# Arlo0o/StereoScene

Hardware: AMD Instinct MI355X
Metric: voxels/sec fwd+bwd, 256x256x32 grid D=192 (higher is better)
Workload: dtype f32; 1 GPU; kitti_d192: stereo pair features 2x[B,640,48,160] -> 256x256x32 occupancy, D=192, fwd+bwd incl. 4 losses; batch_per_gpu=1, global_batch=1, parallelism=dp1, train_mode=True

## Files before the change

include/ssbev.h:

```cpp
#ifndef SSBEV_H
#define SSBEV_H

#include <stddef.h>
#include <stdint.h>

#ifdef __cplusplus
extern "C" {
#endif

#define SSBEV_OK 0
#define SSBEV_EINVAL (-1)
#define SSBEV_EWORKSPACE (-2)
#define SSBEV_ELAUNCH (-3)

typedef void* ssbev_stream_t;

int ssbev_version(void);
const char* ssbev_build_arch(void);
void ssbev_env_refresh(void);

typedef struct {
  int B;
  int P;
  int C;
// ... 39 lines not shown
typedef struct { int B, C, G, D, H, W; float down; int align_corners; } ssbev_gwc_dims;
int ssbev_gwc_warp_fwd(const float* left, const float* right, const float* calib, float* vol,
                       const ssbev_gwc_dims* d, ssbev_stream_t stream);
int ssbev_gwc_warp_bwd(const float* grad_vol, const float* left, const float* right,
                       const float* calib, float* grad_left, float* grad_right,
                       const ssbev_gwc_dims* d, ssbev_stream_t stream);
size_t ssbev_gwc_warp_bwd_workspace(const ssbev_gwc_dims* d);
int ssbev_gwc_warp_bwd_fused(const float* grad_vol, const float* left, const float* right,
                             const float* calib, float* grad_left, float* grad_right,
                             const ssbev_gwc_dims* d, void* workspace, size_t ws_bytes, ssbev_stream_t stream);

typedef struct {
  int B, Cin, Cout;
  int Di, Hi, Wi;
  int Do, Ho, Wo;
  int kd, kh, kw;
  int sd, sh, sw;
  int pd, ph, pw;
  int dd, dh, dw;
  int transposed;
  int relu;
  int accumulate;
  int tile_hint;
  int precision;
} ssbev_conv_dims;

size_t ssbev_conv_packed_weight_elems(const ssbev_conv_dims* d);
int ssbev_conv_kernel_class(const ssbev_conv_dims* d, int mode);

size_t ssbev_conv_thin_workspace(const ssbev_conv_dims* d, int mode);
size_t ssbev_conv_thin_packed_elems(const ssbev_conv_dims* d, int mode);
int ssbev_conv_thin_pack(const float* w_src, float* w_packed, const ssbev_conv_dims* d, int mode, ssbev_stream_t stream);
int ssbev_conv_thin_run(const float* x, const float* w_packed, const float* bias, float* y, const ssbev_conv_dims* d,
                        int mode, void* workspace, size_t ws_bytes, ssbev_stream_t stream);
int ssbev_conv_pack_weight(const float* w_src, float* w_packed, const ssbev_conv_dims* d, int mode,
                           ssbev_stream_t stream);
int ssbev_conv_fwd(const float* x, const float* w_packed, const float* bias, float* y,
                   const ssbev_conv_dims* d, ssbev_stream_t stream);
int ssbev_conv_fwd_bf16(const uint16_t* x, const float* w_packed, const float* bias, void* y,
                        const ssbev_conv_dims* d, ssbev_stream_t stream);
int ssbev_conv_bwd_data_bf16(const uint16_t* gy, const float* w_packed_t, void* gx,
                             const ssbev_conv_dims* d, ssbev_stream_t stream);
int ssbev_conv_bwd_weight_bf16(const uint16_t* x, const uint16_t* gy, float* gw, const ssbev_conv_dims* d,
                               void* ws, size_t ws_bytes, ssbev_stream_t stream);
int ssbev_conv_bwd_data(const float* gy, const float* w_packed_t, float* gx,
                        const ssbev_conv_dims* d, ssbev_stream_t stream);
size_t ssbev_conv_bwd_weight_workspace(const ssbev_conv_dims* d);
int ssbev_conv_bwd_weight(const float* x, const float* gy, float* gw, const ssbev_conv_dims* d,
                          void* ws, size_t ws_bytes, ssbev_stream_t stream);

typedef struct { int M, N, K, batch; int out_fp32; } ssbev_gemm16_dims;
size_t ssbev_gemm16_packed_elems(const ssbev_gemm16_dims* d);
int ssbev_gemm16_pack(const float* B, uint16_t* packed, const ssbev_gemm16_dims* d, ssbev_stream_t stream);
int ssbev_gemm16_nn(const uint16_t* A, const uint16_t* packed, void* C, const ssbev_gemm16_dims* d, ssbev_stream_t stream);
size_t ssbev_gemm16_tn_workspace(const ssbev_gemm16_dims* d);
int ssbev_gemm16_tn(const uint16_t* A, const uint16_t* B, float* C, const ssbev_gemm16_dims* d, float* workspace,
                    size_t workspace_elems, ssbev_stream_t stream);

typedef struct { int B, C, G; int64_t S; float eps; int relu; int stats_given; int pre_act; int64_t ld_y, ld_gy; int io_dtype; } ssbev_norm_dims;
size_t ssbev_groupnorm_workspace(const ssbev_norm_dims* d);
int ssbev_groupnorm_fwd(const float* x, const float* gamma, const float* beta, const float* residual,
                        float* y, float* mean, float* rstd, const ssbev_norm_dims* d, void* ws,
                        size_t ws_bytes, ssbev_stream_t stream);
int ssbev_groupnorm_bwd(const float* gy, const float* x, const float* y, const float* gamma,
                        const float* mean, const float* rstd, float* gx, float* gresidual,
                        float* ggamma, float* gbeta, const ssbev_norm_dims* d, void* ws,
                        size_t ws_bytes, ssbev_stream_t stream);
size_t ssbev_groupnorm_mask_words(const ssbev_norm_dims* d);
int ssbev_groupnorm_fwd_mask(const float* x, const float* gamma, const float* beta, const float* residual, float* y,
                             float* mean, float* rstd, uint64_t* relu_mask, const ssbev_norm_dims* d, void* ws,
                             size_t ws_bytes, ssbev_stream_t stream);
int ssbev_groupnorm_bwd_mask(const float* gy, const float* x, const uint64_t* relu_mask, const float* gamma,
                             const float* mean, const float* rstd, float* gx, float* gresidual, float* ggamma, float* gbeta,
                             const ssbev_norm_dims* d, void* ws, size_t ws_bytes, ssbev_stream_t stream);

typedef struct { float* running_mean; float* running_var; float momentum; int64_t n; } ssbev_norm_ext;
int ssbev_groupnorm_fwd_ext(const float* x, const float* gamma, const float* beta, const float* residual, float* y,
                            float* mean, float* rstd, uint64_t* relu_mask, const ssbev_norm_dims* d,
                            const ssbev_norm_ext* ext, void* ws, size_t ws_bytes, ssbev_stream_t stream);
int ssbev_groupnorm_bwd_ext(const float* gy, const float* x, const float* y, const uint64_t* relu_mask, const float* gamma,
                            const float* mean, const float* rstd, float* gx, float* gresidual, float* ggamma, float* gbeta,
                            const ssbev_norm_dims* d, const ssbev_norm_ext* ext, void* ws, size_t ws_bytes,
                            ssbev_stream_t stream);

typedef struct { int B, C, Ga, Gb; int64_t S; float eps_a, eps_b; int relu; int a_batch, b_batch; int io_dtype;  } ssbev_norm2_dims;
size_t ssbev_groupnorm2_workspace(const ssbev_norm2_dims* d);
int ssbev_groupnorm2_fwd(const float* xa, const float* gamma_a, const float* beta_a, float* mean_a, float* rstd_a,
                         const float* xb, const float* gamma_b, const float* beta_b, float* mean_b, float* rstd_b, float* y,
                         uint64_t* relu_mask, const ssbev_norm2_dims* d, void* ws, size_t ws_bytes, ssbev_stream_t stream);
int ssbev_groupnorm2_bwd(const float* gy, const uint64_t* relu_mask, const float* xa, const float* gamma_a, const float* mean_a,
                         const float* rstd_a, const float* xb, const float* gamma_b, const float* mean_b, const float* rstd_b,
                         float* gxa, float* gxb, float* ggamma_a, float* gbeta_a, float* ggamma_b, float* gbeta_b,
                         const ssbev_norm2_dims* d, void* ws, size_t ws_bytes, ssbev_stream_t stream);

typedef struct { float* running_mean_a; float* running_var_a; float momentum_a;
                 float* running_mean_b; float* running_var_b; float momentum_b; } ssbev_norm2_ext;
int ssbev_groupnorm2_fwd_ext(const float* xa, const float* gamma_a, const float* beta_a, float* mean_a, float* rstd_a,
                             const float* xb, const float* gamma_b, const float* beta_b, float* mean_b, float* rstd_b, float* y,
                             uint64_t* relu_mask, const ssbev_norm2_dims* d, const ssbev_norm2_ext* ext, void* ws, size_t ws_bytes,
                             ssbev_stream_t stream);
int ssbev_groupnorm2_bwd_ext(const float* gy, const uint64_t* relu_mask, const float* xa, const float* gamma_a, const float* mean_a,
                             const float* rstd_a, const float* xb, const float* gamma_b, const float* mean_b, const float* rstd_b,
                             float* gxa, float* gxb, float* ggamma_a, float* gbeta_a, float* ggamma_b, float* gbeta_b,
                             const ssbev_norm2_dims* d, const ssbev_norm2_ext* ext, void* ws, size_t ws_bytes,
                             ssbev_stream_t stream);

typedef struct { int B, D, H, W, C; } ssbev_upsample_dims;
int ssbev_trilinear2x_fwd(const float* x, float* y, const ssbev_upsample_dims* d, ssbev_stream_t stream);
int ssbev_trilinear2x_bwd(const float* gy, float* gx, const ssbev_upsample_dims* d, ssbev_stream_t stream);

typedef struct { float lr, beta1, beta2, eps, weight_decay, max_grad_norm; int step; } ssbev_adamw_cfg;
size_t ssbev_grad_norm_workspace(void);
int ssbev_grad_norm(const float* g, int64_t n, float* norm_out, void* ws, size_t ws_bytes,
                    ssbev_stream_t stream);
int ssbev_adamw_step(float* p, const float* g, float* m, float* v, int64_t n,
                     const ssbev_adamw_cfg* c, const float* grad_norm, ssbev_stream_t stream);

typedef struct { int B, D, H, W, C; } ssbev_occloss_dims;
int ssbev_occ_loss_num_sums(void);
size_t ssbev_occ_loss_workspace(const ssbev_occloss_dims* d);
int ssbev_occ_loss_fwd(const float* logits, const uint8_t* label, const float* class_weight, double* sums,
                       const ssbev_occloss_dims* d, void* ws, size_t ws_bytes, ssbev_stream_t stream);
int ssbev_bri_shell_chunks(void);
int ssbev_bri_shell_pre_fwd(const float* q, const float* kv, const float* conf, const float* wq, const float* bq,
                            const float* wk, const float* bk, const float* wv, const float* bv, float* Q, float* K, float* Vc,
                            int B, int D, int T, ssbev_stream_t stream);
int ssbev_bri_shell_post_fwd(const float* out, const float* kv, const float* gamma, float* y, int B, int D, int T,
                             ssbev_stream_t stream);
int ssbev_bri_shell_post_bwd(const float* gy, const float* out, const float* gamma, float* gout, float* delta_part, double* part,
                             int B, int D, int T, ssbev_stream_t stream);
int ssbev_bri_shell_pre_bwd(const float* gQ, const float* gK, const float* gVc, const float* q, const float* kv, const float* conf,
                            const float* gres, const float* wq, const float* wk, const float* wv, const float* bv, float* gq,
                            float* gkv, float* gconf_part, double* part, int B, int D, int T, ssbev_stream_t stream);

int ssbev_occ_loss_tail(const double* sums, float w_ce, float w_sem, float w_geo, float* out5, double* jac,
                        ssbev_stream_t stream);
size_t ssbev_occ_loss_bwd_workspace(const ssbev_occloss_dims* d);
int ssbev_occ_loss_bwd(const float* logits, const uint8_t* label, const float* class_weight,
                       const float* coef, float* grad_logits, const ssbev_occloss_dims* d, void* ws,
                       size_t ws_bytes, ssbev_stream_t stream);

int ssbev_bn_update_running(const float* mean, const float* rstd, float* running_mean, float* running_var, int C,
                            float momentum, float eps, int64_t n, ssbev_stream_t stream);

int ssbev_softmax_axis_fwd(const float* x, float* y, int64_t outer, int C, int64_t inner, ssbev_stream_t stream);
int ssbev_softmax_axis_bwd(const float* y, const float* gy, float* gx, int64_t outer, int C, int64_t inner,
                           ssbev_stream_t stream);
int ssbev_softmax_rows_fwd(const float* x, float* y, int64_t rows, int C, ssbev_stream_t stream);
int ssbev_softmax_rows_bwd(const float* y, const float* gy, float* gx, int64_t rows, int C, ssbev_stream_t stream);

typedef struct { int B, C, H, W, G, k, pad, dil; } ssbev_dcn_dims;
int ssbev_dcn_im2col(const float* x, const float* offset, float* cols, const ssbev_dcn_dims* d, ssbev_stream_t stream);
size_t ssbev_dcn_col2im_workspace(const ssbev_dcn_dims* d);
int ssbev_dcn_col2im(const float* x, const float* offset, const float* gcols, float* gx, float* goffset,
                     const ssbev_dcn_dims* d, void* ws, size_t ws_bytes, ssbev_stream_t stream);

int ssbev_resize_pil_u8(const uint8_t* src, int Hs, int Ws, int C, const int32_t* kk_h, const int32_t* bounds_h, int ksize_h,
                        const int32_t* kk_v, const int32_t* bounds_v, int ksize_v, uint8_t* tmp, uint8_t* dst, int Hd, int Wd,
                        ssbev_stream_t stream);
int ssbev_crop_normalize_u8(const uint8_t* src, int Hs, int Ws, float* dst, int x0, int y0, int w, int h, int flip,
                            const float* mean, const float* stdinv, int swap_rb, ssbev_stream_t stream);
int ssbev_crop_rotate_normalize_u8(const uint8_t* src, int Hs, int Ws, float* dst, int x0, int y0, int w, int h, int flip,
                                   const int32_t* affine6, const float* mean, const float* stdinv, int swap_rb,
                                   ssbev_stream_t stream);
size_t ssbev_depth_bce_workspace(int BN, int fH, int fW);
int ssbev_depth_bce_fwd(const float* gt_depths, const float* depth_pred, float* out2, int BN, int D, int fH, int fW, int ds,
                        float c0, float dd, float weight, void* ws, size_t ws_bytes, ssbev_stream_t stream);
int ssbev_depth_bce_bwd(const float* depth_pred, const float* grad_loss, const float* out2, float* grad_pred, int BN, int D, int fH,
                        int fW, int ds, float c0, float dd, float weight, const void* ws, ssbev_stream_t stream);

size_t ssbev_lidar_depth_workspace(int H, int W);
int ssbev_lidar_depth_map(const float* points, int n_points, const float* cam, const float* labels, float* uvd,
                          unsigned char* valid, float* depth, float* seg, int H, int W, void* ws, size_t ws_bytes,
                          ssbev_stream_t stream);

typedef struct { int B, C, Hi, Wi, Ho, Wo, k, stride, pad_t, pad_l; } ssbev_dw_dims;
int ssbev_dwconv2d_fwd(const float* x, const float* w, float* y, const ssbev_dw_dims* d, ssbev_stream_t stream);
int ssbev_dwconv2d_bwd_data(const float* gy, const float* w, float* gx, const ssbev_dw_dims* d, ssbev_stream_t stream);
size_t ssbev_dwconv2d_bwd_weight_workspace(const ssbev_dw_dims* d);
int ssbev_dwconv2d_bwd_weight(const float* x, const float* gy, float* gw, const ssbev_dw_dims* d, float* ws,
                              size_t ws_elems, ssbev_stream_t stream);
int ssbev_swish_fwd(const float* x, float* y, int64_t n, ssbev_stream_t stream);
int ssbev_swish_bwd(const float* x, const float* gy, float* gx, int64_t n, ssbev_stream_t stream);
size_t ssbev_chan_sum_workspace(int B, int64_t S, int C);
int ssbev_chan_sum(const float* a, const float* bmul, float* out, int B, int64_t S, int C, float scale, float* ws,
                   size_t ws_elems, ssbev_stream_t stream);
int ssbev_chan_scale(const float* x, const float* gate, float* y, int B, int64_t S, int C, float scale,
                     ssbev_stream_t stream);

typedef struct { int B, D, H, W, C; } ssbev_wino_dims;
int ssbev_wino_input_transform(const float* x, float* V, const ssbev_wino_dims* d, ssbev_stream_t stream);
int ssbev_wino_output_transform(const float* M, float* y, const ssbev_wino_dims* d, ssbev_stream_t stream);
int ssbev_wino_output_adjoint(const float* gy, float* Z, const ssbev_wino_dims* d, ssbev_stream_t stream);
int ssbev_wino2d_input_transform(const float* x, float* V, const ssbev_wino_dims* d, ssbev_stream_t stream);
int ssbev_wino2d_output_transform(const float* M, float* y, const ssbev_wino_dims* d, ssbev_stream_t stream);
int ssbev_wino2d_output_adjoint(const float* gy, float* Z, const ssbev_wino_dims* d, ssbev_stream_t stream);
int ssbev_wino_input_transform_bf16(const float* x, uint16_t* V, const ssbev_wino_dims* d, ssbev_stream_t stream);
int ssbev_wino_output_transform_bf16(const uint16_t* M, float* y, const ssbev_wino_dims* d, ssbev_stream_t stream);
int ssbev_wino_output_adjoint_bf16(const float* gy, uint16_t* Z, const ssbev_wino_dims* d, ssbev_stream_t stream);
int ssbev_wino2d_input_transform_bf16(const float* x, uint16_t* V, const ssbev_wino_dims* d, ssbev_stream_t stream);
int ssbev_wino2d_output_transform_bf16(const uint16_t* M, float* y, const ssbev_wino_dims* d, ssbev_stream_t stream);
int ssbev_wino2d_output_adjoint_bf16(const float* gy, uint16_t* Z, const ssbev_wino_dims* d, ssbev_stream_t stream);
int ssbev_wino_input_transform_bf16a(const uint16_t* x, uint16_t* V, const ssbev_wino_dims* d, ssbev_stream_t stream);
int ssbev_wino_output_transform_bf16a(const uint16_t* M, uint16_t* y, const ssbev_wino_dims* d, ssbev_stream_t stream);
int ssbev_wino_output_adjoint_bf16a(const uint16_t* gy, uint16_t* Z, const ssbev_wino_dims* d, ssbev_stream_t stream);
int ssbev_wino2d_input_transform_bf16a(const uint16_t* x, uint16_t* V, const ssbev_wino_dims* d, ssbev_stream_t stream);
int ssbev_wino2d_output_transform_bf16a(const uint16_t* M, uint16_t* y, const ssbev_wino_dims* d, ssbev_stream_t stream);
int ssbev_wino2d_output_adjoint_bf16a(const uint16_t* gy, uint16_t* Z, const ssbev_wino_dims* d, ssbev_stream_t stream);
int ssbev_wino43_input_transform(const float* x, float* V, const ssbev_wino_dims* d, ssbev_stream_t stream);
int ssbev_wino43_output_transform(const float* M, float* y, const ssbev_wino_dims* d, ssbev_stream_t stream);
int ssbev_wino43_output_adjoint(const float* gy, float* Z, const ssbev_wino_dims* d, ssbev_stream_t stream);
int ssbev_wino43_2d_input_transform(const float* x, float* V, const ssbev_wino_dims* d, ssbev_stream_t stream);
int ssbev_wino43_2d_output_transform(const float* M, float* y, const ssbev_wino_dims* d, ssbev_stream_t stream);
int ssbev_wino43_2d_output_transform_acc(const float* M, float* y, const ssbev_wino_dims* d, ssbev_stream_t stream);
int ssbev_wino2d_output_transform_acc(const float* M, float* y, const ssbev_wino_dims* d, ssbev_stream_t stream);
int ssbev_wino43_2d_output_adjoint(const float* gy, float* Z, const ssbev_wino_dims* d, ssbev_stream_t stream);
int ssbev_wino43_input_transform_bf16(const float* x, uint16_t* V, const ssbev_wino_dims* d, ssbev_stream_t stream);
int ssbev_wino43_output_transform_bf16(const uint16_t* M, float* y, const ssbev_wino_dims* d, ssbev_stream_t stream);
int ssbev_wino43_output_adjoint_bf16(const float* gy, uint16_t* Z, const ssbev_wino_dims* d, ssbev_stream_t stream);
int ssbev_wino43_2d_input_transform_bf16(const float* x, uint16_t* V, const ssbev_wino_dims* d, ssbev_stream_t stream);
int ssbev_wino43_2d_output_transform_bf16(const uint16_t* M, float* y, const ssbev_wino_dims* d, ssbev_stream_t stream);
int ssbev_wino43_2d_output_adjoint_bf16(const float* gy, uint16_t* Z, const ssbev_wino_dims* d, ssbev_stream_t stream);
int ssbev_wino444_input_transform(const float* x, float* V, const ssbev_wino_dims* d, ssbev_stream_t stream);
int ssbev_wino444_output_transform(const float* M, float* y, const ssbev_wino_dims* d, ssbev_stream_t stream);
int ssbev_wino444_output_adjoint(const float* gy, float* Z, const ssbev_wino_dims* d, ssbev_stream_t stream);
int ssbev_wino43_weight_transform(const float* w, float* U, int Cout, int Cin, int ndim, int mode, ssbev_stream_t stream);
int ssbev_wino43_weight_grad(const float* gU, float* gw, int Cout, int Cin, int ndim, ssbev_stream_t stream);
int ssbev_wino_weight_transform(const float* w, float* U, int Cout, int Cin, int ndim, int mode, ssbev_stream_t stream);
int ssbev_wino_weight_grad(const float* gU, float* gw, int Cout, int Cin, int ndim, ssbev_stream_t stream);
size_t ssbev_wino_dgemm_packed_elems(int Cout, int Cin);
int ssbev_wino_dgemm_pack(const float* w, float* Wp, int Cout, int Cin, int mode, ssbev_stream_t stream);
int ssbev_wino_dgemm(const float* P, const float* Wp, float* Mo, const ssbev_wino_dims* d, int N, ssbev_stream_t stream);
int ssbev_wino_bgemm(const float* A, const float* Wp, float* Cm, int64_t T, int K, int N, ssbev_stream_t stream);

typedef struct {
  int M, N, K, batch;
  int64_t lda, ldb, ldc, sa, sb, sc;
  int relu;
  int d2s_D, d2s_H, d2s_W, d2s_kd, d2s_kh, d2s_kw, d2s_Co;
  const int64_t* d2s_rowoff;
  const float* ep_mul;
  const float* ep_rowsub;
} ssbev_gemm_dims;
int ssbev_gemm_d2s_rowoff(int64_t* rowoff, int M, int D, int H, int W, int kd, int kh, int kw, int Co, ssbev_stream_t stream);
size_t ssbev_gemm_nn_workspace(const ssbev_gemm_dims* d);
size_t ssbev_gemm_nt_workspace(const ssbev_gemm_dims* d);
int ssbev_gemm_nn(const float* A, const float* B, const float* bias, float* C, const ssbev_gemm_dims* d, void* workspace,
                  size_t ws_bytes, ssbev_stream_t stream);
int ssbev_gemm_nt(const float* A, const float* W, const float* bias, float* C, const ssbev_gemm_dims* d, void* workspace,
                  size_t ws_bytes, ssbev_stream_t stream);
size_t ssbev_gemm_tn_workspace(const ssbev_gemm_dims* d);
int ssbev_gemm_tn(const float* A, const float* B, float* C, const ssbev_gemm_dims* d, void* workspace, size_t ws_bytes,
                  ssbev_stream_t stream);

int ssbev_wino43_df_supported(const ssbev_wino_dims* d, int N);
int ssbev_wino43_df_instance(const ssbev_wino_dims* d, int N);
size_t ssbev_wino43_df_packed_elems(int Cout, int Cin);
int ssbev_wino43_df_pack(const float* w, float* Wp, int Cout, int Cin, int mode, ssbev_stream_t stream);
int ssbev_wino43_df_gemm(const float* P, const float* Wp, float* Mo, const ssbev_wino_dims* d, int N, ssbev_stream_t stream);
size_t ssbev_wino43_df_wgrad_workspace(const ssbev_wino_dims* d, int N);
int ssbev_wino43_df_wgrad(const float* P, const float* Z, float* gw, const ssbev_wino_dims* d, int N, void* workspace,
                          size_t ws_bytes, ssbev_stream_t stream);

#ifdef __cplusplus
}
#endif
#endif
```

stereoscene_amd/capi.py:

```python
import ctypes as C
import os

import torch

_HERE = os.path.dirname(os.path.abspath(__file__))
LIB_PATH = os.path.join(_HERE, "_lib", "libssbev_hip.so")

OK, EINVAL, EWORKSPACE, ELAUNCH = 0, -1, -2, -3
_ERR = {EINVAL: "SSBEV_EINVAL (bad dims / null pointer / unsupported configuration)",
        EWORKSPACE: "SSBEV_EWORKSPACE (workspace too small)",
        ELAUNCH: "SSBEV_ELAUNCH (HIP launch failure)"}


class SsbevError(RuntimeError):
    pass


class PoolDims(C.Structure):
    _fields_ = [("B", C.c_int), ("P", C.c_int), ("C", C.c_int), ("nx", C.c_int), ("ny", C.c_int), ("nz", C.c_int),
                ("origin", C.c_float * 3), ("dx", C.c_float * 3)]


class LiftDims(C.Structure):
    _fields_ = [("N", C.c_int), ("D", C.c_int), ("HW", C.c_int)]
# ... 37 lines not shown
class Norm2Ext(C.Structure):
    _fields_ = [("running_mean_a", C.c_void_p), ("running_var_a", C.c_void_p), ("momentum_a", C.c_float),
                ("running_mean_b", C.c_void_p), ("running_var_b", C.c_void_p), ("momentum_b", C.c_float)]


class DcnDims(C.Structure):
    _fields_ = [(n, C.c_int) for n in ("B", "C", "H", "W", "G", "k", "pad", "dil")]


class DwDims(C.Structure):
    _fields_ = [(n, C.c_int) for n in ("B", "C", "Hi", "Wi", "Ho", "Wo", "k", "stride", "pad_t", "pad_l")]


class WinoDims(C.Structure):
    _fields_ = [(n, C.c_int) for n in ("B", "D", "H", "W", "C")]


class UpsampleDims(C.Structure):
    _fields_ = [("B", C.c_int), ("D", C.c_int), ("H", C.c_int), ("W", C.c_int), ("C", C.c_int)]


class GemmDims(C.Structure):
    _fields_ = [("M", C.c_int), ("N", C.c_int), ("K", C.c_int), ("batch", C.c_int),
                ("lda", C.c_int64), ("ldb", C.c_int64), ("ldc", C.c_int64), ("sa", C.c_int64), ("sb", C.c_int64), ("sc", C.c_int64),
                ("relu", C.c_int),
                ("d2s_D", C.c_int), ("d2s_H", C.c_int), ("d2s_W", C.c_int), ("d2s_kd", C.c_int), ("d2s_kh", C.c_int),
                ("d2s_kw", C.c_int), ("d2s_Co", C.c_int), ("d2s_rowoff", C.c_void_p),
                ("ep_mul", C.c_void_p), ("ep_rowsub", C.c_void_p)]


class AdamWCfg(C.Structure):
    _fields_ = [("lr", C.c_float), ("beta1", C.c_float), ("beta2", C.c_float), ("eps", C.c_float),
                ("weight_decay", C.c_float), ("max_grad_norm", C.c_float), ("step", C.c_int)]


_P = C.c_void_p
SIGNATURES = {
    "ssbev_version": (C.c_int, []),
    "ssbev_build_arch": (C.c_char_p, []),
    "ssbev_env_refresh": (None, []),
    "ssbev_voxel_index": (C.c_int, [_P, _P, _P, C.POINTER(PoolDims), _P]),
    "ssbev_coords_to_vox": (C.c_int, [_P, C.c_int, _P, C.POINTER(PoolDims), _P]),
    "ssbev_pool_prepare_workspace": (C.c_size_t, [C.c_int, C.POINTER(PoolDims)]),
    "ssbev_pool_prepare": (C.c_int, [_P, C.c_int, _P, _P, C.POINTER(PoolDims), _P, C.c_size_t, _P]),
    "ssbev_pool_long_list_elems": (C.c_size_t, [C.c_int]),
    "ssbev_pool_prepare2": (C.c_int, [_P, C.c_int, _P, _P, _P, C.POINTER(PoolDims), _P, C.c_size_t, _P]),
    "ssbev_bev_pool_fwd": (C.c_int, [_P, _P, _P, _P, C.POINTER(PoolDims), _P]),
    "ssbev_bev_pool_bwd": (C.c_int, [_P, _P, C.c_int, _P, C.POINTER(PoolDims), _P]),
    "ssbev_lift_splat_fwd": (C.c_int, [_P, _P, _P, _P, _P, C.POINTER(PoolDims), C.POINTER(LiftDims), _P]),
    "ssbev_lift_splat_fwd2": (C.c_int, [_P, _P, _P, _P, _P, _P, C.POINTER(PoolDims), C.POINTER(LiftDims), _P]),
    "ssbev_lift_splat_bwd": (C.c_int, [_P, _P, _P, _P, _P, _P, C.POINTER(PoolDims), C.POINTER(LiftDims), _P]),
    "ssbev_gwc_warp_fwd": (C.c_int, [_P, _P, _P, _P, C.POINTER(GwcDims), _P]),
    "ssbev_gwc_warp_bwd": (C.c_int, [_P, _P, _P, _P, _P, _P, C.POINTER(GwcDims), _P]),
    "ssbev_gwc_warp_bwd_workspace": (C.c_size_t, [C.POINTER(GwcDims)]),
    "ssbev_gwc_warp_bwd_fused": (C.c_int, [_P, _P, _P, _P, _P, _P, C.POINTER(GwcDims), _P, C.c_size_t, _P]),
    "ssbev_conv_packed_weight_elems": (C.c_size_t, [C.POINTER(ConvDims)]),
    "ssbev_conv_kernel_class": (C.c_int, [C.POINTER(ConvDims), C.c_int]),
    "ssbev_frustum_geometry": (C.c_int, [_P] * 9 + [C.POINTER(GeomDims), _P]),
    "ssbev_conv_pack_weight": (C.c_int, [_P, _P, C.POINTER(ConvDims), C.c_int, _P]),
    "ssbev_conv_thin_workspace": (C.c_size_t, [C.POINTER(ConvDims), C.c_int]),
    "ssbev_conv_thin_packed_elems": (C.c_size_t, [C.POINTER(ConvDims), C.c_int]),
    "ssbev_conv_thin_pack": (C.c_int, [_P, _P, C.POINTER(ConvDims), C.c_int, _P]),
    "ssbev_conv_thin_run": (C.c_int, [_P, _P, _P, _P, C.POINTER(ConvDims), C.c_int, _P, C.c_size_t, _P]),
    "ssbev_conv_fwd": (C.c_int, [_P, _P, _P, _P, C.POINTER(ConvDims), _P]),
    "ssbev_conv_bwd_data": (C.c_int, [_P, _P, _P, C.POINTER(ConvDims), _P]),
    "ssbev_conv_fwd_bf16": (C.c_int, [_P, _P, _P, _P, C.POINTER(ConvDims), _P]),
    "ssbev_conv_bwd_data_bf16": (C.c_int, [_P, _P, _P, C.POINTER(ConvDims), _P]),
    "ssbev_conv_bwd_weight_bf16": (C.c_int, [_P, _P, _P, C.POINTER(ConvDims), _P, C.c_size_t, _P]),
    "ssbev_conv_bwd_weight_workspace": (C.c_size_t, [C.POINTER(ConvDims)]),
    "ssbev_conv_bwd_weight": (C.c_int, [_P, _P, _P, C.POINTER(ConvDims), _P, C.c_size_t, _P]),
    "ssbev_gemm16_packed_elems": (C.c_size_t, [C.POINTER(Gemm16Dims)]),
    "ssbev_gemm16_pack": (C.c_int, [_P, _P, C.POINTER(Gemm16Dims), _P]),
    "ssbev_gemm16_nn": (C.c_int, [_P, _P, _P, C.POINTER(Gemm16Dims), _P]),
    "ssbev_gemm16_tn_workspace": (C.c_size_t, [C.POINTER(Gemm16Dims)]),
    "ssbev_gemm16_tn": (C.c_int, [_P, _P, _P, C.POINTER(Gemm16Dims), _P, C.c_size_t, _P]),
    "ssbev_groupnorm_workspace": (C.c_size_t, [C.POINTER(NormDims)]),
    "ssbev_groupnorm_fwd": (C.c_int, [_P] * 7 + [C.POINTER(NormDims), _P, C.c_size_t, _P]),
    "ssbev_groupnorm_bwd": (C.c_int, [_P] * 10 + [C.POINTER(NormDims), _P, C.c_size_t, _P]),
    "ssbev_groupnorm_mask_words": (C.c_size_t, [C.POINTER(NormDims)]),
    "ssbev_groupnorm_fwd_mask": (C.c_int, [_P] * 8 + [C.POINTER(NormDims), _P, C.c_size_t, _P]),
    "ssbev_groupnorm_bwd_mask": (C.c_int, [_P] * 10 + [C.POINTER(NormDims), _P, C.c_size_t, _P]),
    "ssbev_groupnorm_fwd_ext": (C.c_int, [_P] * 8 + [C.POINTER(NormDims), C.POINTER(NormExt), _P, C.c_size_t, _P]),
    "ssbev_groupnorm_bwd_ext": (C.c_int, [_P] * 11 + [C.POINTER(NormDims), C.POINTER(NormExt), _P, C.c_size_t, _P]),
    "ssbev_groupnorm2_fwd_ext": (C.c_int, [_P] * 12 + [C.POINTER(Norm2Dims), C.POINTER(Norm2Ext), _P, C.c_size_t, _P]),
    "ssbev_groupnorm2_bwd_ext": (C.c_int, [_P] * 16 + [C.POINTER(Norm2Dims), C.POINTER(Norm2Ext), _P, C.c_size_t, _P]),
    "ssbev_groupnorm2_workspace": (C.c_size_t, [C.POINTER(Norm2Dims)]),
    "ssbev_groupnorm2_fwd": (C.c_int, [_P] * 12 + [C.POINTER(Norm2Dims), _P, C.c_size_t, _P]),
    "ssbev_groupnorm2_bwd": (C.c_int, [_P] * 16 + [C.POINTER(Norm2Dims), _P, C.c_size_t, _P]),
    "ssbev_trilinear2x_fwd": (C.c_int, [_P, _P, C.POINTER(UpsampleDims), _P]),
    "ssbev_trilinear2x_bwd": (C.c_int, [_P, _P, C.POINTER(UpsampleDims), _P]),
    "ssbev_dcn_im2col": (C.c_int, [_P, _P, _P, C.POINTER(DcnDims), _P]),
    "ssbev_dcn_col2im_workspace": (C.c_size_t, [C.POINTER(DcnDims)]),
    "ssbev_dcn_col2im": (C.c_int, [_P, _P, _P, _P, _P, C.POINTER(DcnDims), _P, C.c_size_t, _P]),
    "ssbev_bn_update_running": (C.c_int, [_P, _P, _P, _P, C.c_int, C.c_float, C.c_float, C.c_int64, _P]),
    "ssbev_resize_pil_u8": (C.c_int, [_P, C.c_int, C.c_int, C.c_int, _P, _P, C.c_int, _P, _P, C.c_int, _P, _P, C.c_int, C.c_int, _P]),
    "ssbev_crop_normalize_u8": (C.c_int, [_P, C.c_int, C.c_int, _P, C.c_int, C.c_int, C.c_int, C.c_int, C.c_int, _P, _P, C.c_int, _P]),
    "ssbev_crop_rotate_normalize_u8": (C.c_int, [_P, C.c_int, C.c_int, _P, C.c_int, C.c_int, C.c_int, C.c_int, C.c_int, _P, _P, _P,
                                                C.c_int, _P]),
    "ssbev_depth_bce_workspace": (C.c_size_t, [C.c_int, C.c_int, C.c_int]),
    "ssbev_depth_bce_fwd": (C.c_int, [_P, _P, _P] + [C.c_int] * 5 + [C.c_float] * 3 + [_P, C.c_size_t, _P]),
    "ssbev_depth_bce_bwd": (C.c_int, [_P, _P, _P, _P] + [C.c_int] * 5 + [C.c_float] * 3 + [_P, _P]),
    "ssbev_lidar_depth_workspace": (C.c_size_t, [C.c_int, C.c_int]),
    "ssbev_lidar_depth_map": (C.c_int, [_P, C.c_int, _P, _P, _P, _P, _P, _P, C.c_int, C.c_int, _P, C.c_size_t, _P]),
    "ssbev_dwconv2d_fwd": (C.c_int, [_P, _P, _P, C.POINTER(DwDims), _P]),
    "ssbev_dwconv2d_bwd_data": (C.c_int, [_P, _P, _P, C.POINTER(DwDims), _P]),
    "ssbev_dwconv2d_bwd_weight_workspace": (C.c_size_t, [C.POINTER(DwDims)]),
    "ssbev_dwconv2d_bwd_weight": (C.c_int, [_P, _P, _P, C.POINTER(DwDims), _P, C.c_size_t, _P]),
    "ssbev_swish_fwd": (C.c_int, [_P, _P, C.c_int64, _P]),
    "ssbev_swish_bwd": (C.c_int, [_P, _P, _P, C.c_int64, _P]),
    "ssbev_chan_sum_workspace": (C.c_size_t, [C.c_int, C.c_int64, C.c_int]),
    "ssbev_chan_sum": (C.c_int, [_P, _P, _P, C.c_int, C.c_int64, C.c_int, C.c_float, _P, C.c_size_t, _P]),
    "ssbev_chan_scale": (C.c_int, [_P, _P, _P, C.c_int, C.c_int64, C.c_int, C.c_float, _P]),
    "ssbev_wino_input_transform": (C.c_int, [_P, _P, C.POINTER(WinoDims), _P]),
    "ssbev_wino_output_transform": (C.c_int, [_P, _P, C.POINTER(WinoDims), _P]),
    "ssbev_wino_output_adjoint": (C.c_int, [_P, _P, C.POINTER(WinoDims), _P]),
    "ssbev_wino_weight_transform": (C.c_int, [_P, _P, C.c_int, C.c_int, C.c_int, C.c_int, _P]),
    "ssbev_wino_weight_grad": (C.c_int, [_P, _P, C.c_int, C.c_int, C.c_int, _P]),
    "ssbev_wino_dgemm_packed_elems": (C.c_size_t, [C.c_int, C.c_int]),
    "ssbev_wino_dgemm_pack": (C.c_int, [_P, _P, C.c_int, C.c_int, C.c_int, _P]),
    "ssbev_wino_dgemm": (C.c_int, [_P, _P, _P, C.POINTER(WinoDims), C.c_int, _P]),
    "ssbev_wino_bgemm": (C.c_int, [_P, _P, _P, C.c_int64, C.c_int, C.c_int, _P]),
    "ssbev_gemm_d2s_rowoff": (C.c_int, [_P, C.c_int, C.c_int, C.c_int, C.c_int, C.c_int, C.c_int, C.c_int, C.c_int, _P]),
    "ssbev_gemm_nn_workspace": (C.c_size_t, [C.POINTER(GemmDims)]),
    "ssbev_gemm_nt_workspace": (C.c_size_t, [C.POINTER(GemmDims)]),
    "ssbev_gemm_nn": (C.c_int, [_P, _P, _P, _P, C.POINTER(GemmDims), _P, C.c_size_t, _P]),
    "ssbev_gemm_nt": (C.c_int, [_P, _P, _P, _P, C.POINTER(GemmDims), _P, C.c_size_t, _P]),
    "ssbev_gemm_tn_workspace": (C.c_size_t, [C.POINTER(GemmDims)]),
    "ssbev_gemm_tn": (C.c_int, [_P, _P, _P, C.POINTER(GemmDims), _P, C.c_size_t, _P]),
    "ssbev_wino43_df_supported": (C.c_int, [C.POINTER(WinoDims), C.c_int]),
    "ssbev_wino43_df_instance": (C.c_int, [C.POINTER(WinoDims), C.c_int]),
    "ssbev_wino43_df_packed_elems": (C.c_size_t, [C.c_int, C.c_int]),
    "ssbev_wino43_df_pack": (C.c_int, [_P, _P, C.c_int, C.c_int, C.c_int, _P]),
    "ssbev_wino43_df_gemm": (C.c_int, [_P, _P, _P, C.POINTER(WinoDims), C.c_int, _P]),
    "ssbev_wino43_df_wgrad_workspace": (C.c_size_t, [C.POINTER(WinoDims), C.c_int]),
    "ssbev_wino43_df_wgrad": (C.c_int, [_P, _P, _P, C.POINTER(WinoDims), C.c_int, _P, C.c_size_t, _P]),
    "ssbev_wino2d_input_transform": (C.c_int, [_P, _P, C.POINTER(WinoDims), _P]),
    "ssbev_wino2d_output_transform": (C.c_int, [_P, _P, C.POINTER(WinoDims), _P]),
    "ssbev_wino2d_output_adjoint": (C.c_int, [_P, _P, C.POINTER(WinoDims), _P]),
    "ssbev_wino43_input_transform": (C.c_int, [_P, _P, C.POINTER(WinoDims), _P]),
    "ssbev_wino43_input_transform_bf16": (C.c_int, [_P, _P, C.POINTER(WinoDims), _P]),
    "ssbev_wino43_output_transform": (C.c_int, [_P, _P, C.POINTER(WinoDims), _P]),
    "ssbev_wino43_output_transform_bf16": (C.c_int, [_P, _P, C.POINTER(WinoDims), _P]),
    "ssbev_wino43_output_adjoint": (C.c_int, [_P, _P, C.POINTER(WinoDims), _P]),
    "ssbev_wino43_output_adjoint_bf16": (C.c_int, [_P, _P, C.POINTER(WinoDims), _P]),
    "ssbev_wino43_2d_input_transform": (C.c_int, [_P, _P, C.POINTER(WinoDims), _P]),
    "ssbev_wino43_2d_input_transform_bf16": (C.c_int, [_P, _P, C.POINTER(WinoDims), _P]),
    "ssbev_wino43_2d_output_transform": (C.c_int, [_P, _P, C.POINTER(WinoDims), _P]),
    "ssbev_wino43_2d_output_transform_acc": (C.c_int, [_P, _P, C.POINTER(WinoDims), _P]),
    "ssbev_wino2d_output_transform_acc": (C.c_int, [_P, _P, C.POINTER(WinoDims), _P]),
    "ssbev_wino43_2d_output_transform_bf16": (C.c_int, [_P, _P, C.POINTER(WinoDims), _P]),
    "ssbev_wino43_2d_output_adjoint": (C.c_int, [_P, _P, C.POINTER(WinoDims), _P]),
    "ssbev_wino43_2d_output_adjoint_bf16": (C.c_int, [_P, _P, C.POINTER(WinoDims), _P]),
    "ssbev_wino444_input_transform": (C.c_int, [_P, _P, C.POINTER(WinoDims), _P]),
    "ssbev_wino444_output_transform": (C.c_int, [_P, _P, C.POINTER(WinoDims), _P]),
    "ssbev_wino444_output_adjoint": (C.c_int, [_P, _P, C.POINTER(WinoDims), _P]),
    "ssbev_wino43_weight_transform": (C.c_int, [_P, _P, C.c_int, C.c_int, C.c_int, C.c_int, _P]),
    "ssbev_wino43_weight_grad": (C.c_int, [_P, _P, C.c_int, C.c_int, C.c_int, _P]),
    "ssbev_wino_input_transform_bf16": (C.c_int, [_P, _P, C.POINTER(WinoDims), _P]),
    "ssbev_wino_output_transform_bf16": (C.c_int, [_P, _P, C.POINTER(WinoDims), _P]),
    "ssbev_wino_output_adjoint_bf16": (C.c_int, [_P, _P, C.POINTER(WinoDims), _P]),
    "ssbev_wino2d_input_transform_bf16": (C.c_int, [_P, _P, C.POINTER(WinoDims), _P]),
    "ssbev_wino2d_output_transform_bf16": (C.c_int, [_P, _P, C.POINTER(WinoDims), _P]),
    "ssbev_wino2d_output_adjoint_bf16": (C.c_int, [_P, _P, C.POINTER(WinoDims), _P]),
    "ssbev_wino_input_transform_bf16a": (C.c_int, [_P, _P, C.POINTER(WinoDims), _P]),
    "ssbev_wino_output_transform_bf16a": (C.c_int, [_P, _P, C.POINTER(WinoDims), _P]),
    "ssbev_wino_output_adjoint_bf16a": (C.c_int, [_P, _P, C.POINTER(WinoDims), _P]),
    "ssbev_wino2d_input_transform_bf16a": (C.c_int, [_P, _P, C.POINTER(WinoDims), _P]),
    "ssbev_wino2d_output_transform_bf16a": (C.c_int, [_P, _P, C.POINTER(WinoDims), _P]),
    "ssbev_wino2d_output_adjoint_bf16a": (C.c_int, [_P, _P, C.POINTER(WinoDims), _P]),
    "ssbev_softmax_axis_fwd": (C.c_int, [_P, _P, C.c_int64, C.c_int, C.c_int64, _P]),
    "ssbev_softmax_axis_bwd": (C.c_int, [_P, _P, _P, C.c_int64, C.c_int, C.c_int64, _P]),
    "ssbev_softmax_rows_fwd": (C.c_int, [_P, _P, C.c_int64, C.c_int, _P]),
    "ssbev_softmax_rows_bwd": (C.c_int, [_P, _P, _P, C.c_int64, C.c_int, _P]),
    "ssbev_occ_loss_num_sums": (C.c_int, []),
    "ssbev_occ_loss_workspace": (C.c_size_t, [C.POINTER(UpsampleDims)]),
    "ssbev_occ_loss_fwd": (C.c_int, [_P, _P, _P, _P, C.POINTER(UpsampleDims), _P, C.c_size_t, _P]),
    "ssbev_occ_loss_tail": (C.c_int, [_P, C.c_float, C.c_float, C.c_float, _P, _P, _P]),
    "ssbev_bri_shell_chunks": (C.c_int, []),
    "ssbev_bri_shell_pre_fwd": (C.c_int, [_P] * 12 + [C.c_int] * 3 + [_P]),
    "ssbev_bri_shell_post_fwd": (C.c_int, [_P] * 4 + [C.c_int] * 3 + [_P]),
    "ssbev_bri_shell_post_bwd": (C.c_int, [_P] * 6 + [C.c_int] * 3 + [_P]),
    "ssbev_bri_shell_pre_bwd": (C.c_int, [_P] * 15 + [C.c_int] * 3 + [_P]),
    "ssbev_occ_loss_bwd_workspace": (C.c_size_t, [C.POINTER(UpsampleDims)]),
    "ssbev_occ_loss_bwd": (C.c_int, [_P, _P, _P, _P, _P, C.POINTER(UpsampleDims), _P, C.c_size_t, _P]),
    "ssbev_grad_norm_workspace": (C.c_size_t, []),
    "ssbev_grad_norm": (C.c_int, [_P, C.c_int64, _P, _P, C.c_size_t, _P]),
    "ssbev_adamw_step": (C.c_int, [_P, _P, _P, _P, C.c_int64, C.POINTER(AdamWCfg), _P, _P]),
}

_lib = None


def load():
    global _lib
    if _lib is None:
        if not os.path.exists(LIB_PATH):
            raise SsbevError(f"{LIB_PATH} is missing: run `python -m stereoscene_amd.build` "
                             "(there is no CPU / PyTorch fallback for the HIP operators)")
        lib = C.CDLL(LIB_PATH)
        for name, (res, args) in SIGNATURES.items():
            fn = getattr(lib, name)
            fn.restype, fn.argtypes = res, args
        _lib = lib
    return _lib


def check(code, what):
    if code != OK:
        raise SsbevError(f"{what}: {_ERR.get(code, code)}")


def ptr(t):
    if t is None:
        return None
    if not t.is_cuda:
        raise SsbevError("ssbev operators run on the MI355X only: got a CPU tensor (no CPU fallback exists)")
    if not t.is_contiguous():
        raise SsbevError("ssbev operators need contiguous buffers")
    return C.c_void_p(t.data_ptr())


_raw_stream = getattr(torch._C, "_cuda_getCurrentRawStream", None)


def stream():
    if _raw_stream is not None:
        return C.c_void_p(_raw_stream(torch.cuda.current_device()))
    return C.c_void_p(torch.cuda.current_stream().cuda_stream)
```

stereoscene_amd/csrc/groupnorm.hip:

```cpp
#include "common.h"

#include <algorithm>

namespace {

constexpr int NT = 256;
constexpr int PNT = 256;
constexpr int kStatBlocks = 768;
constexpr int kSlabLanes = 8;

struct GnGeom {
  int B, C, G;
  long S;
  int chunks;
  long chunk_len;
  float eps;
  int relu;
  int slab_q;
  int pre;
  long ldy, ldg;
};

__device__ __forceinline__ void gelu_both(float x, float& u, float& du) {
  const float z = fabsf(x) * 0.70710678118654752f;
// ... 137 lines not shown
    for (int k = 0; k < VW; ++k) {
      lds[((size_t)r * Cs + c4 * VW + k) * 2 + 0] = a0[k];
      lds[((size_t)r * Cs + c4 * VW + k) * 2 + 1] = a1[k];
    }
  }
  __syncthreads();
  for (int t = tid; t < Cs; t += PNT) {
    float s0 = 0.0f, s1 = 0.0f;
    for (int rr = 0; rr < rows; ++rr) { s0 += lds[((size_t)rr * Cs + t) * 2]; s1 += lds[((size_t)rr * Cs + t) * 2 + 1]; }
    st_record(partial + ((size_t)(b * g.chunks + chunk) * g.C + q0 * VW + t) * 2, s0, s1);
  }
}

constexpr int FT = 1024;

__device__ __forceinline__ double wave_sum_d(double v) {
#pragma unroll
  for (int off = 32; off > 0; off >>= 1) v += __shfl_xor(v, off, 64);
  return v;
}
__device__ __forceinline__ void block_sum2(double& a, double& q, double* s0, double* s1) {
  a = wave_sum_d(a); q = wave_sum_d(q);
  const int w = threadIdx.x >> 6;
  if ((threadIdx.x & 63) == 0) { s0[w] = a; s1[w] = q; }
  __syncthreads();
  double ta = 0.0, tq = 0.0;
#pragma unroll
  for (int i = 0; i < FT / 64; ++i) { ta += s0[i]; tq += s1[i]; }
  a = ta; q = tq;
}

template <typename T>
__global__ void __launch_bounds__(FT)
gn_finalize_fwd_kernel(const float* __restrict__ partial, const T* __restrict__ x, float* __restrict__ mean,
                       float* __restrict__ rstd, GnGeom g) {
  __shared__ double s0[FT], s1[FT];
  __shared__ float piv[FT];
  const int b = blockIdx.x / g.G, grp = blockIdx.x % g.G;
  const int cpg = g.C / g.G, n_el = g.chunks * cpg;
  const bool lds_piv = cpg <= FT;
  constexpr int kFinBatch = 16;
  float pf_own = 0.0f;
  if (lds_piv && (int)threadIdx.x < cpg) pf_own = ld1(x + (size_t)b * g.S * g.C + grp * cpg + threadIdx.x);
  double a[4] = {0, 0, 0, 0}, q[4] = {0, 0, 0, 0};
  bool first = true;
  for (int i0 = threadIdx.x; i0 < n_el || first; i0 += kFinBatch * FT) {
    float2 rec[kFinBatch];
#pragma unroll
    for (int k = 0; k < kFinBatch; ++k) {
      const int i = i0 + k * FT;
      rec[k] = make_float2(0.f, 0.f);
      if (i < n_el) {
        const int chunk = i / cpg, c = grp * cpg + i % cpg;
        rec[k] = *reinterpret_cast<const float2*>(partial + ((size_t)(b * g.chunks + chunk) * g.C + c) * 2);
      }
    }
    if (first) {
      if (lds_piv && (int)threadIdx.x < cpg) piv[threadIdx.x] = g.pre ? gelu_f(pf_own) : pf_own;
      __syncthreads();
      first = false;
    }
#pragma unroll
    for (int k = 0; k < kFinBatch; ++k) {
      const int i = i0 + k * FT;
      if (i < n_el) {
        const int chunk = i / cpg, c = grp * cpg + i % cpg;
        float pf = lds_piv ? piv[i % cpg] : ld1(x + (size_t)b * g.S * g.C + c);
        if (!lds_piv && g.pre) pf = gelu_f(pf);
        const double pd = pf;
        const double n = (double)(min(g.S, (long)(chunk + 1) * g.chunk_len) - (long)chunk * g.chunk_len);
        a[k & 3] += (double)rec[k].x + n * pd;
        q[k & 3] += (double)rec[k].y + 2.0 * pd * (double)rec[k].x + n * pd * pd;
      }
    }
  }
  double sa = (a[0] + a[1]) + (a[2] + a[3]), sq = (q[0] + q[1]) + (q[2] + q[3]);
  block_sum2(sa, sq, s0, s1);
  if (threadIdx.x == 0) {
    const double n = (double)g.S * cpg;
    const double m = sa / n;
    double var = sq / n - m * m;
    if (var < 0.0) var = 0.0;
    mean[blockIdx.x] = (float)m;
    rstd[blockIdx.x] = (float)(1.0 / sqrt(var + (double)g.eps));
  }
}

template <typename T>
__global__ void __launch_bounds__(256)
bn_finalize_fwd_flat_kernel(const float* __restrict__ partial, const T* __restrict__ x, float* __restrict__ mean,
                            float* __restrict__ rstd, GnGeom g, float* __restrict__ rm, float* __restrict__ rv, float mom,
                            float unbias) {
  const int i = blockIdx.x * 4 + (threadIdx.x >> 6), lane = threadIdx.x & 63;
  if (i >= g.B * g.C) return;
  const int b = i / g.C, c = i % g.C;
  double a = 0.0, q = 0.0;
  float pf = ld1(x + (size_t)b * g.S * g.C + c);
  constexpr int kFlatBatch = 12;
  for (int chunk0 = lane; chunk0 < g.chunks; chunk0 += 64 * kFlatBatch) {
    float2 rec[kFlatBatch];
#pragma unroll
    for (int k = 0; k < kFlatBatch; ++k) {
      const int chunk = chunk0 + 64 * k;
      rec[k] = chunk < g.chunks ? *reinterpret_cast<const float2*>(partial + ((size_t)(b * g.chunks + chunk) * g.C + c) * 2)
                                : make_float2(0.f, 0.f);
    }
#pragma unroll
    for (int k = 0; k < kFlatBatch; ++k) { a += rec[k].x; q += rec[k].y; }
  }
  a = wave_sum_d(a); q = wave_sum_d(q);
  if (lane == 0) {
    if (g.pre) pf = gelu_f(pf);
    const double n = (double)g.S, md = a / n;
    double var = q / n - md * md;
    if (var < 0.0) var = 0.0;
    const double m = (double)pf + md;
    const float mf = (float)m, rs = (float)(1.0 / sqrt(var + (double)g.eps));
    mean[i] = mf;
    rstd[i] = rs;
    if (rm && b == 0) {
      const float vf = 1.0f / (rs * rs) - g.eps;
      rm[c] = (1.0f - mom) * rm[c] + mom * mf;
      rv[c] = (1.0f - mom) * rv[c] + mom * (vf * unbias);
    }
  }
}

__global__ void __launch_bounds__(256)
bn_finalize_bwd_flat_kernel(const float* __restrict__ partial, const float* __restrict__ gamma, float* __restrict__ coef,
                            float* __restrict__ dgamma, float* __restrict__ dbeta, GnGeom g) {
  const int c = blockIdx.x * 4 + (threadIdx.x >> 6), lane = threadIdx.x & 63;
  if (c >= g.C) return;
  double tb = 0.0, ts = 0.0;
  const double gm = gamma[c], n = (double)g.S;
  for (int b = 0; b < g.B; ++b) {
    double sb = 0.0, ss = 0.0;
    constexpr int kFlatBatch = 12;
    for (int chunk0 = lane; chunk0 < g.chunks; chunk0 += 64 * kFlatBatch) {
      float2 rec[kFlatBatch];
#pragma unroll
      for (int k = 0; k < kFlatBatch; ++k) {
        const int chunk = chunk0 + 64 * k;
        rec[k] = chunk < g.chunks ? *reinterpret_cast<const float2*>(partial + ((size_t)(b * g.chunks + chunk) * g.C + c) * 2)
                                  : make_float2(0.f, 0.f);
      }
#pragma unroll
      for (int k = 0; k < kFlatBatch; ++k) { sb += rec[k].x; ss += rec[k].y; }
    }
    sb = wave_sum_d(sb); ss = wave_sum_d(ss);
    if (lane == 0) {
      coef[(b * g.C + c) * 2 + 0] = (float)(gm * ss / n);
      coef[(b * g.C + c) * 2 + 1] = (float)(gm * sb / n);
    }
    tb += sb; ts += ss;
  }
  if (lane == 0) { dbeta[c] = (float)tb; dgamma[c] = (float)ts; }
}

__device__ __forceinline__ void relu_mask_store4(unsigned long long* __restrict__ mask, long i, const float (&v)[4]) {
  unsigned long long bal[4];
#pragma unroll
  for (int k = 0; k < 4; ++k) bal[k] = __ballot(v[k] > 0.0f);
  const int ln = threadIdx.x & 63;
  const unsigned long long act = __ballot(1);
  if (act == ~0ull || __popcll(act) >= 4) {
    if (ln < 4) {
// ... 542 lines not shown
                       (const T*)nullptr, nullptr, nullptr, nullptr, partial, g);
  else
    hipLaunchKernelGGL((gn_partial_kernel<0, false, 0, T, VW>), grid, dim3(PNT), lds, st, x, (const T*)nullptr,
                       (const T*)nullptr, nullptr, nullptr, nullptr, partial, g);
  if (g.G == g.C) {
    const bool run = ext && ext->running_mean && ext->running_var;
    hipLaunchKernelGGL(bn_finalize_fwd_flat_kernel<T>, dim3(cdiv((size_t)g.B * g.C, 4)), dim3(256), 0, st, partial, x, mean, rstd, g,
                       run ? ext->running_mean : nullptr, run ? ext->running_var : nullptr, run ? ext->momentum : 0.0f,
                       run ? (float)((double)ext->n / (double)(ext->n > 1 ? ext->n - 1 : 1)) : 0.0f);
  } else {
    hipLaunchKernelGGL(gn_finalize_fwd_kernel<T>, dim3(g.B * g.G), dim3(FT), 0, st, partial, x, mean, rstd, g);
  }
  return SSBEV_OK;
}

template <typename T, int VW>
static int groupnorm_fwd_t(const T* x, const float* gamma, const float* beta, const T* residual, T* y,
                           float* mean, float* rstd, unsigned long long* mask, const ssbev_norm_dims* d, void* ws,
                           ssbev_stream_t stream, const ssbev_norm_ext* ext = nullptr) {
  const GnGeom g = make_geom(d);
  hipStream_t st = as_stream(stream);
  float* partial = static_cast<float*>(ws);
  if (!d->stats_given) {
    const int rc = gn_stats_fwd<T, VW>(x, mean, rstd, g, partial, ext, st);
    if (rc != SSBEV_OK) return rc;
  }
  const long totalv = (long)g.B * g.S * (g.C / 4);
  const unsigned blocks = apply_blocks(totalv, g.C / 4);
  if (g.pre)
    hipLaunchKernelGGL((gn_apply_fwd_kernel<true, T, 4>), dim3(blocks), dim3(NT), 0, st, x, gamma, beta, residual, mean, rstd, y,
                       d->relu ? mask : nullptr, g, totalv);
  else
    hipLaunchKernelGGL((gn_apply_fwd_kernel<false, T, 4>), dim3(blocks), dim3(NT), 0, st, x, gamma, beta, residual, mean, rstd, y,
                       d->relu ? mask : nullptr, g, totalv);
  return ssbev_launch_status();
}
}

static bool gn_rows16(const ssbev_norm_dims* d, const void* const* ptrs, int n) {
  if ((d->ld_y != 0 && d->ld_y % 8 != 0) || (d->ld_gy != 0 && d->ld_gy % 8 != 0)) return false;
  for (int i = 0; i < n; ++i)
    if (ptrs[i] && reinterpret_cast<uintptr_t>(ptrs[i]) % 16 != 0) return false;
  return true;
}

static int groupnorm_fwd_impl(const float* x, const float* gamma, const float* beta, const float* residual, float* y,
                              float* mean, float* rstd, unsigned long long* mask, const ssbev_norm_dims* d, void* ws,
                              size_t ws_bytes, ssbev_stream_t stream, const ssbev_norm_ext* ext = nullptr) {
  if (!gn_ok(d) || !x || !gamma || !beta || !y || !mean || !rstd || !ws) return SSBEV_EINVAL;
  if (residual && d->ld_y != 0 && d->ld_y != d->C) return SSBEV_EINVAL;
  if (ws_bytes < ssbev_groupnorm_workspace(d)) return SSBEV_EWORKSPACE;
  if (d->io_dtype == 1) {
    const bf16_t* x16 = reinterpret_cast<const bf16_t*>(x);
    const bf16_t* r16 = reinterpret_cast<const bf16_t*>(residual);
    bf16_t* y16 = reinterpret_cast<bf16_t*>(y);
    if (gn_vw(1, d->C) == 8) {
      const void* ps[1] = {x};
      if (!gn_rows16(d, ps, 1)) return groupnorm_fwd_t<bf16_t, 4>(x16, gamma, beta, r16, y16, mean, rstd, mask, d, ws, stream, ext);
      return groupnorm_fwd_t<bf16_t, 8>(x16, gamma, beta, r16, y16, mean, rstd, mask, d, ws, stream, ext);
    }
    return groupnorm_fwd_t<bf16_t, 4>(x16, gamma, beta, r16, y16, mean, rstd, mask, d, ws, stream, ext);
  }
  return groupnorm_fwd_t<float, 4>(x, gamma, beta, residual, y, mean, rstd, mask, d, ws, stream, ext);
}

int ssbev_groupnorm_fwd_ext(const float* x, const float* gamma, const float* beta, const float* residual, float* y,
                            float* mean, float* rstd, uint64_t* relu_mask, const ssbev_norm_dims* d,
                            const ssbev_norm_ext* ext, void* ws, size_t ws_bytes, ssbev_stream_t stream) {
  return groupnorm_fwd_impl(x, gamma, beta, residual, y, mean, rstd, reinterpret_cast<unsigned long long*>(relu_mask), d, ws,
                            ws_bytes, stream, ext);
}

int ssbev_groupnorm_fwd(const float* x, const float* gamma, const float* beta, const float* residual, float* y,
                        float* mean, float* rstd, const ssbev_norm_dims* d, void* ws, size_t ws_bytes,
                        ssbev_stream_t stream) {
  return groupnorm_fwd_impl(x, gamma, beta, residual, y, mean, rstd, nullptr, d, ws, ws_bytes, stream);
}

int ssbev_groupnorm_fwd_mask(const float* x, const float* gamma, const float* beta, const float* residual, float* y,
                             float* mean, float* rstd, uint64_t* relu_mask, const ssbev_norm_dims* d, void* ws,
                             size_t ws_bytes, ssbev_stream_t stream) {
  if (d && d->relu && !relu_mask) return SSBEV_EINVAL;
  return groupnorm_fwd_impl(x, gamma, beta, residual, y, mean, rstd, reinterpret_cast<unsigned long long*>(relu_mask), d, ws,
                            ws_bytes, stream);
}

int ssbev_bn_update_running(const float* mean, const float* rstd, float* running_mean, float* running_var, int C,
                            float momentum, float eps, int64_t n, ssbev_stream_t stream) {
  if (!mean || !rstd || !running_mean || !running_var || C <= 0 || n <= 0) return SSBEV_EINVAL;
  hipLaunchKernelGGL(bn_update_running_kernel, dim3(cdiv((size_t)C, 256)), dim3(256), 0, as_stream(stream), mean, rstd,
                     running_mean, running_var, C, momentum, eps, (float)((double)n / (double)(n > 1 ? n - 1 : 1)));
  return ssbev_launch_status();
}

extern "C++" {
template <typename T, int VW>
static int groupnorm_bwd_t(const T* gy, const T* x, const T* y, const unsigned long long* mask,
                           const float* gamma, const float* mean, const float* rstd, T* gx, T* gresidual,
                           float* ggamma, float* gbeta, const ssbev_norm_dims* d, void* ws, ssbev_stream_t stream,
                           const ssbev_norm_ext* ext = nullptr) {
  const GnGeom g = make_geom(d);
  hipStream_t st = as_stream(stream);
  float* partial = static_cast<float*>(ws);
  float* coef = partial + (size_t)g.B * g.chunks * g.C * 2;
  const size_t lds = lds_bytes(g, VW);
  if (lds > 96 * 1024) return SSBEV_EINVAL;
  {
    const dim3 grid(g.chunks, g.B, gn_slabs(g, VW));
    const int rm = !g.relu ? 0 : (mask ? 1 : 2);
#define SSBEV_GNP(PRE_, RM_) \
    hipLaunchKernelGGL((gn_partial_kernel<1, PRE_, RM_, T, VW>), grid, dim3(PNT), lds, st, x, gy, y, mask, mean, rstd, partial, g)
    if (g.pre) { if (rm == 0) SSBEV_GNP(true, 0); else if (rm == 1) SSBEV_GNP(true, 1); else SSBEV_GNP(true, 2); }
    else { if (rm == 0) SSBEV_GNP(false, 0); else if (rm == 1) SSBEV_GNP(false, 1); else SSBEV_GNP(false, 2); }
#undef SSBEV_GNP
  }
  if (g.G == g.C)
    hipLaunchKernelGGL(bn_finalize_bwd_flat_kernel, dim3(cdiv((size_t)g.C, 4)), dim3(256), 0, st, partial, gamma, coef, ggamma, gbeta, g);
  else
    hipLaunchKernelGGL(gn_finalize_bwd_kernel, dim3(g.B * g.G + g.C), dim3(FT), 0, st, partial, gamma, coef, ggamma, gbeta, g);
  const long totalv = (long)g.B * g.S * (g.C / 4);
  const unsigned blocks = apply_blocks(totalv, g.C / 4);
  if (g.pre)
    hipLaunchKernelGGL((gn_apply_bwd_kernel<true, T, 4>), dim3(blocks), dim3(NT), 0, st, gy, x, y, gamma, mean, rstd, coef, gx,
                       gresidual, mask, g, totalv);
  else
    hipLaunchKernelGGL((gn_apply_bwd_kernel<false, T, 4>), dim3(blocks), dim3(NT), 0, st, gy, x, y, gamma, mean, rstd, coef, gx,
                       gresidual, mask, g, totalv);
  return ssbev_launch_status();
}
}

static int groupnorm_bwd_impl(const float* gy, const float* x, const float* y, const unsigned long long* mask,
                              const float* gamma, const float* mean, const float* rstd, float* gx, float* gresidual,
                              float* ggamma, float* gbeta, const ssbev_norm_dims* d, void* ws, size_t ws_bytes,
                              ssbev_stream_t stream, const ssbev_norm_ext* ext = nullptr) {
  if (!gn_ok(d) || !gy || !x || !gamma || !mean || !rstd || !gx || !ggamma || !gbeta || !ws) return SSBEV_EINVAL;
  if (d->relu && !y && !mask) return SSBEV_EINVAL;
  const bool strided = (d->ld_gy != 0 && d->ld_gy != d->C) || (d->ld_y != 0 && d->ld_y != d->C);
  if (strided && ((d->relu && !mask) || gresidual)) return SSBEV_EINVAL;
  if (ws_bytes < ssbev_groupnorm_workspace(d)) return SSBEV_EWORKSPACE;
  if (d->io_dtype == 1) {
    typedef const bf16_t* cb;
    if (gn_vw(1, d->C) == 8) {
      const void* ps[3] = {gy, x, y};
      if (gn_rows16(d, ps, 3))
        return groupnorm_bwd_t<bf16_t, 8>(reinterpret_cast<cb>(gy), reinterpret_cast<cb>(x), reinterpret_cast<cb>(y), mask, gamma, mean,
                                        rstd, reinterpret_cast<bf16_t*>(gx), reinterpret_cast<bf16_t*>(gresidual), ggamma, gbeta, d, ws,
                                        stream, ext);
    }
    return groupnorm_bwd_t<bf16_t, 4>(reinterpret_cast<cb>(gy), reinterpret_cast<cb>(x), reinterpret_cast<cb>(y), mask, gamma, mean, rstd,
                                      reinterpret_cast<bf16_t*>(gx), reinterpret_cast<bf16_t*>(gresidual), ggamma, gbeta, d, ws, stream, ext);
  }
  return groupnorm_bwd_t<float, 4>(gy, x, y, mask, gamma, mean, rstd, gx, gresidual, ggamma, gbeta, d, ws, stream, ext);
}

int ssbev_groupnorm_bwd_ext(const float* gy, const float* x, const float* y, const uint64_t* relu_mask, const float* gamma,
                            const float* mean, const float* rstd, float* gx, float* gresidual, float* ggamma, float* gbeta,
                            const ssbev_norm_dims* d, const ssbev_norm_ext* ext, void* ws, size_t ws_bytes,
                            ssbev_stream_t stream) {
  return groupnorm_bwd_impl(gy, x, y, reinterpret_cast<const unsigned long long*>(relu_mask), gamma, mean, rstd, gx, gresidual,
                            ggamma, gbeta, d, ws, ws_bytes, stream, ext);
}

int ssbev_groupnorm_bwd(const float* gy, const float* x, const float* y, const float* gamma, const float* mean,
                        const float* rstd, float* gx, float* gresidual, float* ggamma, float* gbeta,
                        const ssbev_norm_dims* d, void* ws, size_t ws_bytes, ssbev_stream_t stream) {
// ... 176 lines not shown
```

stereoscene_amd/csrc/winograd.hip:

```cpp
#include "common.h"

#include <algorithm>
#include <cstdlib>

namespace {

struct WinoGeom { int B, D, H, W, C; int acc = 0; };
__device__ const float kWinoZeros[4] = {0.f, 0.f, 0.f, 0.f};

typedef unsigned short bf16_bits;
__device__ __forceinline__ float fload(const float* p) { return *p; }
__device__ __forceinline__ float fload(const bf16_bits* p) { return __uint_as_float((unsigned)*p << 16); }
__device__ __forceinline__ void fstore(float* p, float v) { *p = v; }
__device__ __forceinline__ void fstore(bf16_bits* p, float v) { *p = __builtin_bit_cast(bf16_bits, (__bf16)v); }

__device__ __forceinline__ void bt4(float* v, int s) {
  const float d0 = v[0], d1 = v[s], d2 = v[2 * s], d3 = v[3 * s];
  v[0] = d0 - d2; v[s] = d1 + d2; v[2 * s] = d2 - d1; v[3 * s] = d1 - d3;
}
__device__ __forceinline__ void a4(float* v, int s) {
  const float g0 = v[0], g1 = v[s];
  v[0] = g0; v[s] = g0 + g1; v[2 * s] = g0 - g1; v[3 * s] = -g1;
}

// ... 467 lines not shown
  for (int a = 0; a < NA; ++a) {
    const int d = DA ? DA * td - 1 + a : 0;
    const long plane = DA ? (long)b * g.D + d : (long)b;
    const bool dok = !DA || (d >= 0 && d < g.D);
#pragma unroll
    for (int e = 0; e < 6; ++e) {
      const int h = 4 * th - 1 + e;
#pragma unroll
      for (int f = 0; f < 6; ++f) {
        const int w = 4 * tw - 1 + f;
        const bool ok = dok && h >= 0 && h < g.H && w >= 0 && w < g.W;
        v[(a * 6 + e) * 6 + f] = ok ? x[((plane * g.H + h) * g.W + w) * g.C + c] : 0.0f;
      }
    }
  }
#pragma unroll
  for (int p = 0; p < NA * 6; ++p) bt6(v + p * 6, 1);
#pragma unroll
  for (int a = 0; a < NA; ++a)
#pragma unroll
    for (int f = 0; f < 6; ++f) bt6(v + a * 36 + f, 6);
  if (DA == 2) {
#pragma unroll
    for (int p = 0; p < 36; ++p) bt4(v + p, 36);
  } else if (DA == 4) {
#pragma unroll
    for (int p = 0; p < 36; ++p) bt6(v + p, 36);
  }
  const long T = total / g.C;
#pragma unroll
  for (int xi = 0; xi < NF; ++xi) fstore(V + ((long)xi * T + tile) * g.C + c, v[xi]);
}

template <int DA, typename TF>
__global__ void __launch_bounds__(256) __attribute__((amdgpu_waves_per_eu(1, DA == 4 ? 1 : (DA == 2 ? 2 : 8))))
wino43_output_kernel(const TF* __restrict__ M, float* __restrict__ y, WinoGeom g, long total) {
  constexpr int NA = DA ? DA + 2 : 1, NF = NA * 36;
  const long i = (long)blockIdx.x * 256 + threadIdx.x;
  if (i >= total) return;
  const int c = (int)(i % g.C);
  const long tile = i / g.C;
  int b, td, th, tw;
  tile43<DA>(tile, g, b, td, th, tw);
  const long T = total / g.C;
  float m[NF];
#pragma unroll
  for (int xi = 0; xi < NF; ++xi) m[xi] = fload(M + ((long)xi * T + tile) * g.C + c);
  float r1[NA * 6 * 4];
#pragma unroll
  for (int p = 0; p < NA * 6; ++p) at6(m + p * 6, 1, r1 + p * 4, 1);
  float r2[NA * 4 * 4];
#pragma unroll
  for (int a = 0; a < NA; ++a)
#pragma unroll
    for (int f = 0; f < 4; ++f) at6(r1 + a * 24 + f, 4, r2 + a * 16 + f, 4);
  if (DA == 0 && g.acc) {
    float oldv[16];
#pragma unroll
    for (int e = 0; e < 4; ++e)
#pragma unroll
      for (int f = 0; f < 4; ++f) oldv[e * 4 + f] = y[(((long)b * g.H + 4 * th + e) * g.W + 4 * tw + f) * g.C + c];
#pragma unroll
    for (int k = 0; k < 16; ++k) r2[k] += oldv[k];
  }
#pragma unroll
  for (int e = 0; e < 4; ++e)
#pragma unroll
    for (int f = 0; f < 4; ++f) {
      if (DA == 2) {
        const float m0 = r2[0 * 16 + e * 4 + f], m1 = r2[1 * 16 + e * 4 + f], m2 = r2[2 * 16 + e * 4 + f], m3 = r2[3 * 16 + e * 4 + f];
        const long base = ((((long)b * g.D + 2 * td) * g.H + 4 * th + e) * g.W + 4 * tw + f) * g.C + c;
        y[base] = m0 + m1 + m2;
        y[base + (long)g.H * g.W * g.C] = m1 - m2 - m3;
      } else if (DA == 4) {
        float o[4];
        at6(r2 + e * 4 + f, 16, o, 1);
        const long base = ((((long)b * g.D + 4 * td) * g.H + 4 * th + e) * g.W + 4 * tw + f) * g.C + c;
#pragma unroll
        for (int a = 0; a < 4; ++a) y[base + (long)a * g.H * g.W * g.C] = o[a];
      } else {
        y[(((long)b * g.H + 4 * th + e) * g.W + 4 * tw + f) * g.C + c] = r2[e * 4 + f];
      }
    }
}

template <int DA, typename TF>
__global__ void __launch_bounds__(256) __attribute__((amdgpu_waves_per_eu(1, DA == 4 ? 1 : (DA == 2 ? 2 : 8))))
wino43_output_adjoint_kernel(const float* __restrict__ gy, TF* __restrict__ Z, WinoGeom g, long total) {
  constexpr int NA = DA ? DA + 2 : 1, NG = DA ? DA : 1, NF = NA * 36;
  const long i = (long)blockIdx.x * 256 + threadIdx.x;
  if (i >= total) return;
  const int c = (int)(i % g.C);
  const long tile = i / g.C;
  int b, td, th, tw;
  tile43<DA>(tile, g, b, td, th, tw);
  float gin[NG * 16];
#pragma unroll
  for (int a = 0; a < NG; ++a) {
    const long plane = DA ? (long)b * g.D + DA * td + a : (long)b;
#pragma unroll
    for (int e = 0; e < 4; ++e)
#pragma unroll
      for (int f = 0; f < 4; ++f) gin[(a * 4 + e) * 4 + f] = gy[((plane * g.H + 4 * th + e) * g.W + 4 * tw + f) * g.C + c];
  }
  float r1[NG * 4 * 6];
#pragma unroll
  for (int p = 0; p < NG * 4; ++p) a6(gin + p * 4, 1, r1 + p * 6, 1);
  float v[NF];
#pragma unroll
  for (int a = 0; a < NG; ++a)
#pragma unroll
    for (int f = 0; f < 6; ++f) a6(r1 + a * 24 + f, 6, v + a * 36 + f, 6);
  if (DA == 2) {
#pragma unroll
    for (int p = 0; p < 36; ++p) a4(v + p, 36);
  } else if (DA == 4) {
#pragma unroll
    for (int p = 0; p < 36; ++p) {
      float t6[6];
      a6(v + p, 36, t6, 1);
#pragma unroll
      for (int a = 0; a < 6; ++a) v[a * 36 + p] = t6[a];
    }
  }
  const long T = total / g.C;
#pragma unroll
  for (int xi = 0; xi < NF; ++xi) fstore(Z + ((long)xi * T + tile) * g.C + c, v[xi]);
}

template <int DA>
__global__ void __launch_bounds__(256)
wino43_weight_kernel(const float* __restrict__ w, float* __restrict__ U, int Cout, int Cin, int mode) {
  constexpr int ND_ = DA ? 3 : 1, TAPS = ND_ * 9, NA = DA ? DA + 2 : 1, NF = NA * 36;
  const int i = blockIdx.x * 256 + threadIdx.x;
  if (i >= Cout * Cin) return;
  const int co = mode == 0 ? i % Cout : i / Cin, ci = mode == 0 ? i / Cout : i % Cin;
  float g[TAPS];
#pragma unroll
  for (int t = 0; t < TAPS; ++t) g[t] = w[((size_t)co * Cin + ci) * TAPS + (mode == 0 ? t : TAPS - 1 - t)];
  float a1[ND_ * 3 * 6];
#pragma unroll
  for (int p = 0; p < ND_ * 3; ++p) g6(g + p * 3, 1, a1 + p * 6, 1);
  float a2[ND_ * 36];
#pragma unroll
  for (int d = 0; d < ND_; ++d)
#pragma unroll
    for (int f = 0; f < 6; ++f) g6(a1 + d * 18 + f, 6, a2 + d * 36 + f, 6);
  float u[NF];
  if (DA == 2) {
#pragma unroll
    for (int p = 0; p < 36; ++p) g4(a2 + p, 36, u + p, 36);
  } else if (DA == 4) {
#pragma unroll
    for (int p = 0; p < 36; ++p) g6(a2 + p, 36, u + p, 36);
  } else {
#pragma unroll
    for (int p = 0; p < 36; ++p) u[p] = a2[p];
  }
  const size_t plane = (size_t)Cout * Cin;
  const size_t pos = mode == 0 ? (size_t)ci * Cout + co : (size_t)co * Cin + ci;
#pragma unroll
  for (int xi = 0; xi < NF; ++xi) U[xi * plane + pos] = u[xi];
}

template <int DA>
__global__ void __launch_bounds__(256)
// ... 314 lines not shown
int ssbev_wino_dgemm_pack(const float* w, float* Wp, int Cout, int Cin, int mode, ssbev_stream_t stream) {
  if (!w || !Wp || Cout <= 0 || Cin <= 0 || (mode != 0 && mode != 1)) return SSBEV_EINVAL;
  const int K = mode == 0 ? Cin : Cout, N = mode == 0 ? Cout : Cin;
  const size_t total = (size_t)((K + 7) & ~7) * ((N + 31) & ~31);
  hipLaunchKernelGGL(wino_weight_packed_kernel, dim3(cdiv(total, 256)), dim3(256), 0, as_stream(stream), w, Wp, Cout, Cin,
                     mode);
  return ssbev_launch_status();
}

int ssbev_wino_dgemm(const float* P, const float* Wp, float* Mo, const ssbev_wino_dims* d, int N, ssbev_stream_t stream) {
  if (!wino_ok(d) || !P || !Wp || !Mo || N <= 0 || d->C % 4 != 0) return SSBEV_EINVAL;
  const WinoGemmGeom g{d->B, d->D, (d->H / 2) * (d->W / 2), d->C, N, (N + 31) & ~31};
  static const int forced = [] { const char* e = ssbev_tune("SSBEV_WINO_TILE"); return e ? atoi(e) : 0; }();
  int mt = 1, nt = 2;
  if (forced) { mt = forced / 10; nt = forced % 10; }
  const int tgroups = (g.Thw + 32 * mt - 1) / (32 * mt), tg4 = (tgroups + 3) >> 2;
  dim3 grid((unsigned)((long)g.B * (g.D / 2) * tg4), cdiv(N, nt * 32), 16), block(256);
  hipStream_t st = as_stream(stream);
#define SSBEV_WG_LAUNCH(M_, N_) hipLaunchKernelGGL((wino_dgemm_kernel<M_, N_>), grid, block, 0, st, P, Wp, Mo, g)
  switch (mt * 10 + nt) {
    case 14: SSBEV_WG_LAUNCH(1, 4); break;
    case 13: SSBEV_WG_LAUNCH(1, 3); break;
    case 12: SSBEV_WG_LAUNCH(1, 2); break;
    case 22: SSBEV_WG_LAUNCH(2, 2); break;
    case 21: SSBEV_WG_LAUNCH(2, 1); break;
    case 11: SSBEV_WG_LAUNCH(1, 1); break;
    default: return SSBEV_EINVAL;
  }
#undef SSBEV_WG_LAUNCH
  return ssbev_launch_status();
}

int ssbev_wino_bgemm(const float* A, const float* Wp, float* Cm, int64_t T, int K, int N, ssbev_stream_t stream) {
  if (!A || !Wp || !Cm || T <= 0 || K <= 0 || N <= 0 || K % 4 != 0) return SSBEV_EINVAL;
  const WinoBgemmGeom g{(long)T, K, N, (N + 31) & ~31};
  const int nt = N > 128 ? 2 : 1;
  const long nrb = ((long)T + kBgBM - 1) / kBgBM;
  const int ycols = cdiv(N, 4 * nt * 32);
  long gx = std::max(1L, (768L + 64 * ycols - 1) / (64 * ycols));
  gx = std::min(gx, std::max(1L, nrb / 4));
  dim3 grid((unsigned)gx, ycols, 64), block(256);
  const size_t lds = (size_t)kBgStages * kBgBM * kBgBK * sizeof(float);
  hipStream_t st = as_stream(stream);
  if (nt == 2) hipLaunchKernelGGL(wino_bgemm_kernel<2>, grid, block, lds, st, A, Wp, Cm, g);
  else hipLaunchKernelGGL(wino_bgemm_kernel<1>, grid, block, lds, st, A, Wp, Cm, g);
  return ssbev_launch_status();
}

SSBEV_WINO2D_ENTRY(ssbev_wino2d_input_transform, wino2d_input_kernel<float>, float, float)
SSBEV_WINO2D_ENTRY(ssbev_wino2d_output_transform, wino2d_output_kernel<float>, float, float)
SSBEV_WINO2D_ENTRY(ssbev_wino2d_output_adjoint, wino2d_output_adjoint_kernel<float>, float, float)

SSBEV_WINO_ENTRY(ssbev_wino_input_transform, wino_input_kernel<float>, float, float)
SSBEV_WINO_ENTRY(ssbev_wino_output_transform, wino_output_kernel<float>, float, float)
SSBEV_WINO_ENTRY(ssbev_wino_output_adjoint, wino_output_adjoint_kernel<float>, float, float)

#define SSBEV_WINO43_ENTRY(NAME, KERNEL, DA, TF, TSRC, TDST)                                                        \
  int NAME(const TSRC* src, TDST* dst, const ssbev_wino_dims* d, ssbev_stream_t stream) {                         \
    if (!wino43_ok(d, DA) || !src || !dst) return SSBEV_EINVAL;                                                     \
    const long total = (long)d->B * (DA ? d->D / DA : d->D) * (d->H / 4) * (d->W / 4) * d->C;                      \
    const WinoGeom g{d->B, d->D, d->H, d->W, d->C};                                                                \
    hipLaunchKernelGGL((KERNEL<DA, TF>), dim3(cdiv((size_t)total, 256)), dim3(256), 0, as_stream(stream), src, dst, g, \
                       total);                                                                                     \
    return ssbev_launch_status();                                                                                  \
  }

SSBEV_WINO43_ENTRY(ssbev_wino43_input_transform, wino43_input_kernel, 2, float, float, float)
SSBEV_WINO43_ENTRY(ssbev_wino43_output_transform, wino43_output_kernel, 2, float, float, float)
SSBEV_WINO43_ENTRY(ssbev_wino43_output_adjoint, wino43_output_adjoint_kernel, 2, float, float, float)
SSBEV_WINO43_ENTRY(ssbev_wino43_2d_input_transform, wino43_input_kernel, 0, float, float, float)
SSBEV_WINO43_ENTRY(ssbev_wino43_2d_output_transform, wino43_output_kernel, 0, float, float, float)
SSBEV_WINO43_ENTRY(ssbev_wino43_2d_output_adjoint, wino43_output_adjoint_kernel, 0, float, float, float)
SSBEV_WINO43_ENTRY(ssbev_wino43_input_transform_bf16, wino43_input_kernel, 2, bf16_bits, float, uint16_t)
SSBEV_WINO43_ENTRY(ssbev_wino43_output_transform_bf16, wino43_output_kernel, 2, bf16_bits, uint16_t, float)
SSBEV_WINO43_ENTRY(ssbev_wino43_output_adjoint_bf16, wino43_output_adjoint_kernel, 2, bf16_bits, float, uint16_t)
SSBEV_WINO43_ENTRY(ssbev_wino43_2d_input_transform_bf16, wino43_input_kernel, 0, bf16_bits, float, uint16_t)
SSBEV_WINO43_ENTRY(ssbev_wino43_2d_output_transform_bf16, wino43_output_kernel, 0, bf16_bits, uint16_t, float)
SSBEV_WINO43_ENTRY(ssbev_wino43_2d_output_adjoint_bf16, wino43_output_adjoint_kernel, 0, bf16_bits, float, uint16_t)

SSBEV_WINO43_ENTRY(ssbev_wino444_input_transform, wino43_input_kernel, 4, float, float, float)
SSBEV_WINO43_ENTRY(ssbev_wino444_output_transform, wino43_output_kernel, 4, float, float, float)
SSBEV_WINO43_ENTRY(ssbev_wino444_output_adjoint, wino43_output_adjoint_kernel, 4, float, float, float)

int ssbev_wino43_2d_output_transform_acc(const float* src, float* dst, const ssbev_wino_dims* d, ssbev_stream_t stream) {
  if (!wino43_ok(d, 0) || !src || !dst) return SSBEV_EINVAL;
  const long total = (long)d->B * d->D * (d->H / 4) * (d->W / 4) * d->C;
  WinoGeom g{d->B, d->D, d->H, d->W, d->C};
  g.acc = 1;
  hipLaunchKernelGGL((wino43_output_kernel<0, float>), dim3(cdiv((size_t)total, 256)), dim3(256), 0, as_stream(stream), src, dst, g, total);
  return ssbev_launch_status();
}

int ssbev_wino2d_output_transform_acc(const float* src, float* dst, const ssbev_wino_dims* d, ssbev_stream_t stream) {
  if (!wino2d_ok(d) || !src || !dst) return SSBEV_EINVAL;
  const long total = (long)d->B * d->D * (d->H / 2) * (d->W / 2) * d->C;
  WinoGeom g{d->B, d->D, d->H, d->W, d->C};
  g.acc = 1;
  hipLaunchKernelGGL(wino2d_output_kernel<float>, dim3(cdiv((size_t)total, 256)), dim3(256), 0, as_stream(stream), src, dst, g, total);
  return ssbev_launch_status();
}

int ssbev_wino43_weight_transform(const float* w, float* U, int Cout, int Cin, int ndim, int mode, ssbev_stream_t stream) {
  if (!w || !U || Cout <= 0 || Cin <= 0 || (ndim != 2 && ndim != 3 && ndim != 4) || (mode != 0 && mode != 1)) return SSBEV_EINVAL;
  const dim3 grid(cdiv((size_t)Cout * Cin, 256)), block(256);
  if (ndim == 4) hipLaunchKernelGGL(wino43_weight_kernel<4>, grid, block, 0, as_stream(stream), w, U, Cout, Cin, mode);
  else if (ndim == 3) hipLaunchKernelGGL(wino43_weight_kernel<2>, grid, block, 0, as_stream(stream), w, U, Cout, Cin, mode);
  else hipLaunchKernelGGL(wino43_weight_kernel<0>, grid, block, 0, as_stream(stream), w, U, Cout, Cin, mode);
  return ssbev_launch_status();
}

int ssbev_wino43_weight_grad(const float* gU, float* gw, int Cout, int Cin, int ndim, ssbev_stream_t stream) {
  if (!gU || !gw || Cout <= 0 || Cin <= 0 || (ndim != 2 && ndim != 3 && ndim != 4)) return SSBEV_EINVAL;
  const dim3 grid(cdiv((size_t)Cout * Cin, 256)), block(256);
  if (ndim == 4) hipLaunchKernelGGL(wino43_weight_grad_kernel<4>, grid, block, 0, as_stream(stream), gU, gw, Cout, Cin);
  else if (ndim == 3) hipLaunchKernelGGL(wino43_weight_grad_kernel<2>, grid, block, 0, as_stream(stream), gU, gw, Cout, Cin);
  else hipLaunchKernelGGL(wino43_weight_grad_kernel<0>, grid, block, 0, as_stream(stream), gU, gw, Cout, Cin);
  return ssbev_launch_status();
}

SSBEV_WINO2D_ENTRY(ssbev_wino2d_input_transform_bf16, wino2d_input_kernel<bf16_bits>, float, uint16_t)
SSBEV_WINO2D_ENTRY(ssbev_wino2d_output_transform_bf16, wino2d_output_kernel<bf16_bits>, uint16_t, float)
SSBEV_WINO2D_ENTRY(ssbev_wino2d_output_adjoint_bf16, wino2d_output_adjoint_kernel<bf16_bits>, float, uint16_t)

#define SSBEV_WINO16_ENTRY(NAME, KERNEL, DIV_D, OK)                                                                   \
  int NAME(const uint16_t* src, uint16_t* dst, const ssbev_wino_dims* d, ssbev_stream_t stream) {                    \
    if (!OK(d) || !src || !dst) return SSBEV_EINVAL;                                                                  \
    const int nv = d->C % 2 == 0 ? 2 : 1;                                                                             \
    const long total = (long)d->B * (d->D / DIV_D) * (d->H / 2) * (d->W / 2) * (d->C / nv);                           \
    const WinoGeom g{d->B, d->D, d->H, d->W, d->C};                                                                   \
    if (nv == 2)                                                                                                      \
      hipLaunchKernelGGL((KERNEL<bf16_bits, bf16_bits, 2>), dim3(cdiv((size_t)total, 256)), dim3(256), 0, as_stream(stream), src, dst, g, total); \
    else                                                                                                              \
      hipLaunchKernelGGL((KERNEL<bf16_bits, bf16_bits, 1>), dim3(cdiv((size_t)total, 256)), dim3(256), 0, as_stream(stream), src, dst, g, total); \
    return ssbev_launch_status();                                                                                     \
  }
SSBEV_WINO16_ENTRY(ssbev_wino_input_transform_bf16a, wino_input_kernel, 2, wino_ok)
SSBEV_WINO16_ENTRY(ssbev_wino_output_transform_bf16a, wino_output_kernel, 2, wino_ok)
SSBEV_WINO16_ENTRY(ssbev_wino_output_adjoint_bf16a, wino_output_adjoint_kernel, 2, wino_ok)
SSBEV_WINO16_ENTRY(ssbev_wino2d_input_transform_bf16a, wino2d_input_kernel, 1, wino2d_ok)
SSBEV_WINO16_ENTRY(ssbev_wino2d_output_transform_bf16a, wino2d_output_kernel, 1, wino2d_ok)
SSBEV_WINO16_ENTRY(ssbev_wino2d_output_adjoint_bf16a, wino2d_output_adjoint_kernel, 1, wino2d_ok)

SSBEV_WINO_ENTRY(ssbev_wino_input_transform_bf16, wino_input_kernel<bf16_bits>, float, uint16_t)
SSBEV_WINO_ENTRY(ssbev_wino_output_transform_bf16, wino_output_kernel<bf16_bits>, uint16_t, float)
SSBEV_WINO_ENTRY(ssbev_wino_output_adjoint_bf16, wino_output_adjoint_kernel<bf16_bits>, float, uint16_t)

}
```

stereoscene_amd/functional.py:

```python
import ctypes as C

import os

import torch

from . import capi, streams



class KernelTimer:

    def __init__(self, families=None):
        self.records = []
        self.counts = {}
        self.families = families

    def span(self, family, flops, nbytes=0.0, tag=None, executed=None):
        c = self.counts.setdefault(family, dict(launches=0, flops=0.0, bytes=0.0, executed=0.0))
        c["launches"] += 1
        c["flops"] += flops
        c["bytes"] += nbytes
        c["executed"] += flops if executed is None else executed
        if self.families is not None and family.split(":")[0] not in self.families:
            return _NOSPAN
# ... 648 lines not shown
            fam = "wgrad_ring16" if (KERNEL_TIMER is not None and lib.ssbev_conv_kernel_class(C.byref(d), 2) == 20) else "wgrad16"
            with _span(fam, conv_flops(d), conv_bytes(d) / 2.0, _conv_tag(d, "wgrad")):
                capi.check(lib.ssbev_conv_bwd_weight_bf16(capi.ptr(xcl), capi.ptr(gcl), capi.ptr(gwp), C.byref(d), capi.ptr(ws),
                                                          ws.numel(), capi.stream()), "ssbev_conv_bwd_weight_bf16")
            return gwp

        gw_side = want_gw and streams.wgrad_on_side(weight)
        want_gb = has_bias and ctx.needs_input_grad[2]
        gb_side = gw_side and want_gb and ctx.bias_leaf
        if gw_side:
            with streams.on_side(gy.device, xcl, gcl) as side:
                gw = weight_gradient()
                if gb_side:
                    gb = gcl.reshape(-1, Cout_g).sum(0, dtype=torch.float32)
                side.publish(gw, gb)
        if want_gx:
            into = _slot_target(ctx.slot, xcl)
            if into is not None:
                d.accumulate = 1
            gxcl = into if into is not None else torch.empty_like(xcl)
            fam = {17: "conv_tap16", 19: "conv_wide16"}.get(lib.ssbev_conv_kernel_class(C.byref(d), 1), "conv_gather16") if KERNEL_TIMER is not None else "conv_gather16"
            with _span(fam, conv_flops(d), conv_bytes(d) / 2.0, _conv_tag(d, "dgrad")):
                wpt = _packed(weight.detach(), d, 1)
                capi.check(lib.ssbev_conv_bwd_data_bf16(capi.ptr(gcl), capi.ptr(wpt), capi.ptr(gxcl), C.byref(d), capi.stream()),
                           "ssbev_conv_bwd_data_bf16")
            d.accumulate = 0
            if ctx.slot is not None:
                ctx.slot.buf = gxcl
            gx = from_cl(gxcl)
        if want_gw and not gw_side:
            gw = weight_gradient()
        if want_gb and not gb_side:
            gb = gcl.reshape(-1, Cout_g).sum(0, dtype=torch.float32)
        return gx, gw, gb, None, None, None, None, None, None, None, None


def _conv16_route(x, weight5, bias, st, pd, dl, transposed, op, relu=False):
    if not (storage_bf16() and x.is_cuda and TILE_HINT in (0, 7, 9)):
        return None
    cin = weight5.shape[0] if transposed else weight5.shape[1]
    cout = weight5.shape[1] if transposed else weight5.shape[0]
    if cin % 8 != 0 or cout % 8 != 0:
        return None
    return _ConvNd16.apply(x, weight5, bias, st, pd, dl, transposed, op, _slot_of(x), bool(relu), False)


WIDE16 = os.environ.get("SSBEV_WIDE16", "1") != "0"
WIDE16_WGRAD = os.environ.get("SSBEV_WIDE16_WGRAD", "direct")


def _wide16_applicable(x, weight, st, pd, dl):
    if x.dim() != 5 or tuple(weight.shape[2:]) != (3, 3, 3) or st != (1, 1, 1) or pd != (1, 1, 1) or dl != (1, 1, 1):
        return False
    if weight.shape[0] % 8 or weight.shape[1] % 8:
        return False
    d = _conv_dims((x.shape[0], x.shape[2], x.shape[3], x.shape[4], x.shape[1]), tuple(weight.shape), st, pd, dl, False, (0, 0, 0))
    d.precision = 2
    return capi.load().ssbev_conv_kernel_class(C.byref(d), 0) == 19


def _wino_wgrad_bf16(xcl, gcl, weight):
    lib = capi.load()
    B, D, H, W, Cin = xcl.shape
    Cout = gcl.shape[-1]
    T = B * (D // 2) * (H // 2) * (W // 2)
    V = _wino_call("ssbev_wino_input_transform_bf16a", xcl, capi.WinoDims(B, D, H, W, Cin), (64, T, Cin), torch.bfloat16)
    Z = _wino_call("ssbev_wino_output_adjoint_bf16a", gcl, capi.WinoDims(B, D, H, W, Cout), (64, T, Cout), torch.bfloat16)
    gU = _bmm16_tn(V, Z)
    gwt = torch.empty(tuple(weight.shape), dtype=torch.float32, device=xcl.device)
    capi.check(lib.ssbev_wino_weight_grad(capi.ptr(gU), capi.ptr(gwt), Cout, Cin, 3, capi.stream()), "ssbev_wino_weight_grad")
    return gwt


def _to_act(y):
    if storage_bf16() and y.dtype == torch.float32 and y.shape[1] % 8 == 0:
        return y.to(torch.bfloat16)
    return y


WINOGRAD = os.environ.get("SSBEV_WINOGRAD", "1") != "0"
WINO_BF16S = os.environ.get("SSBEV_WINO_BF16S", "1") != "0"


def conv3d(x, weight, bias=None, stride=1, padding=0, dilation=1, relu=False):
    st, pd, dl = _triple(stride, 3), _triple(padding, 3), _triple(dilation, 3)
    if storage_bf16() and x.is_cuda and TILE_HINT in (0, 7, 9):
        if WIDE16 and _wide16_applicable(x, weight, st, pd, dl):
            return _ConvNd16.apply(x, weight, bias, st, pd, dl, False, (0, 0, 0), _slot_of(x), bool(relu), False)
        if WINOGRAD and WINO_BF16S and wino_conv3d_applicable(x, weight, st, pd, dl):
            y = _WinoConv.apply(x, weight, _slot_of(x))
            y = y if bias is None else y + _like_act(bias, y).view(1, -1, 1, 1, 1)
            return torch.relu(y) if relu else y
        y = _conv16_route(x, weight, bias, st, pd, dl, False, (0, 0, 0), relu)
        if y is not None:
            return y
        return _to_act(_ConvNd.apply(x, weight, bias, st, pd, dl, False, (0, 0, 0), None, bool(relu)))
    if relu:
        gemm = (GEMM_LAYERS and TILE_HINT == 0 and PRECISION == "fp32" and tuple(weight.shape[2:]) == (1, 1, 1)
                and st == (1, 1, 1) and pd == (0, 0, 0) and weight.shape[1] >= GEMM_MIN_CIN)
        if not x.is_cuda or gemm or (WINOGRAD and TILE_HINT == 0 and wino_conv3d_applicable(x, weight, st, pd, dl)):
            return torch.relu(conv3d(x, weight, bias, stride, padding, dilation))
        return _ConvNd.apply(x, weight, bias, st, pd, dl, False, (0, 0, 0), _slot_of(x), True)
    if (GEMM_LAYERS and TILE_HINT == 0 and PRECISION == "fp32" and x.is_cuda and tuple(weight.shape[2:]) == (1, 1, 1)
            and st == (1, 1, 1) and pd == (0, 0, 0) and weight.shape[1] >= GEMM_MIN_CIN):
        return linear_cl(x, weight, bias)
    if WINOGRAD and TILE_HINT == 0 and wino_conv3d_applicable(x, weight, st, pd, dl):
        B, Cin, D, H, W = x.shape
        if tuple(weight.shape[2:]) == (3, 3, 3) and H % 4 == 0 and W % 4 == 0 and \
                _wino_df_applicable(B, D, H, W, Cin, weight.shape[0]):
            y = _WinoConvDF.apply(x, weight, _slot_of(x))
        else:
            y = _WinoConv.apply(x, weight, _slot_of(x))
        return y if bias is None else y + bias.view(1, -1, 1, 1, 1)
    return _ConvNd.apply(x, weight, bias, st, pd, dl, False, (0, 0, 0), _slot_of(x))


OWN_GEMM = os.environ.get("SSBEV_OWN_GEMM", "1") != "0"
OWN_GEMM_SITES = set(os.environ.get("SSBEV_OWN_GEMM_SITES", "deconv,bri,linear,wino").split(","))


def own_gemm_site(name):
    return OWN_GEMM and ("all" in OWN_GEMM_SITES or name in OWN_GEMM_SITES)


def _rows(t):
    if t.stride(-1) != 1 or (t.dim() == 3 and t.shape[0] > 1 and t.stride(0) % 4 != 0) or t.stride(-2) % 4 != 0 or t.stride(-2) < t.shape[-1]:
        t = t.contiguous()
    if t.data_ptr() % 16:
        t = t.clone(memory_format=torch.contiguous_format)
    return t, t.stride(-2), (t.stride(0) if t.dim() == 3 else 0)


def _rawptr(t):
    return C.c_void_p(t.data_ptr()) if t is not None else None


def _gemm_supported(*ts):
    return OWN_GEMM and all(t.is_cuda and t.dtype == torch.float32 for t in ts)


def _gdims(M, N, K, batch, lda, ldb, ldc, sa, sb, sc, relu=0, d2s=None):
    g = capi.GemmDims(int(M), int(N), int(K), int(batch), int(lda), int(ldb), int(ldc), int(sa), int(sb), int(sc), int(relu),
                      0, 0, 0, 0, 0, 0, 0, None, None, None)
    if d2s is not None:
        (g.d2s_D, g.d2s_H, g.d2s_W, g.d2s_kd, g.d2s_kh, g.d2s_kw, g.d2s_Co), table = d2s
        g.d2s_rowoff = table.data_ptr()
    return g


def gemm_nn(a, b, bias=None, relu=False, tag=None):
    if not _gemm_supported(a, b) or a.shape[-1] % 4 or b.shape[-1] % 4:
        y = torch.matmul(a, b)
        y = y if bias is None else y + bias
        return torch.relu(y) if relu else y
    a, lda, sa = _rows(a)
    b, ldb, sb = _rows(b)
    batch = a.shape[0] if a.dim() == 3 else 1
    M, K, N = a.shape[-2], a.shape[-1], b.shape[-1]
    out = torch.empty(*a.shape[:-1], N, dtype=torch.float32, device=a.device)
    g = _gdims(M, N, K, batch, lda, ldb, N, sa, sb if b.dim() == 3 else 0, M * N, relu)
    fl = 2.0 * batch * M * N * K
    lib = capi.load()
    ws = _ws(lib.ssbev_gemm_nn_workspace(C.byref(g)), a.device)
    with _span("gemm_own", fl, 4.0 * (a.numel() + b.numel() + out.numel()), tag or f"nn {batch}x{M}x{K}x{N}"):
        capi.check(lib.ssbev_gemm_nn(_rawptr(a), _rawptr(b), _rawptr(bias.contiguous() if bias is not None else None),
                                     capi.ptr(out), C.byref(g), capi.ptr(ws), ws.numel(), capi.stream()), "ssbev_gemm_nn")
    return out


def gemm_nt(a, w, bias=None, relu=False, tag=None):
    if not _gemm_supported(a, w) or a.shape[-1] % 4 or w.shape[-2] % 4:
        y = torch.matmul(a, w.transpose(-1, -2))
        y = y if bias is None else y + bias
        return torch.relu(y) if relu else y
    a, lda, sa = _rows(a)
    w, ldb, sb = _rows(w)
    batch = a.shape[0] if a.dim() == 3 else 1
    M, K, N = a.shape[-2], a.shape[-1], w.shape[-2]
    out = torch.empty(*a.shape[:-1], N, dtype=torch.float32, device=a.device)
    g = _gdims(M, N, K, batch, lda, ldb, N, sa, sb if w.dim() == 3 else 0, M * N, relu)
    fl = 2.0 * batch * M * N * K
    lib = capi.load()
    ws = _ws(lib.ssbev_gemm_nt_workspace(C.byref(g)), a.device)
    with _span("gemm_own", fl, 4.0 * (a.numel() + w.numel() + out.numel()), tag or f"nt {batch}x{M}x{K}x{N}"):
        capi.check(lib.ssbev_gemm_nt(_rawptr(a), _rawptr(w), _rawptr(bias.contiguous() if bias is not None else None),
                                     capi.ptr(out), C.byref(g), capi.ptr(ws), ws.numel(), capi.stream()), "ssbev_gemm_nt")
    return out


def gemm_tn(a, b, tag=None, ep_mul=None, ep_rowsub=None):
    if not _gemm_supported(a, b) or a.shape[-1] % 4 or b.shape[-1] % 4:
        c = torch.matmul(a.transpose(-1, -2), b)
        return c if ep_mul is None else ep_mul * (c - ep_rowsub.unsqueeze(-1))
# ... 279 lines not shown
    N = b16.shape[2]
    d = capi.Gemm16Dims(M, N, K, Bt, 1)
    if (K % 8 or N % 8 or a16.dtype != torch.bfloat16 or b16.dtype != torch.bfloat16 or tuple(b16.shape[:2]) != (Bt, M)
            or Bt >= 65536):
        return None
    a16, b16 = a16.contiguous(), b16.contiguous()
    out = torch.empty(Bt, K, N, dtype=torch.float32, device=a16.device)
    ws = torch.empty(max(int(lib.ssbev_gemm16_tn_workspace(C.byref(d))), 4), dtype=torch.float32, device=a16.device)
    with _span("gemm16", 2.0 * Bt * M * K * N, 2.0 * (a16.numel() + b16.numel()) + 4.0 * out.numel(), tag or f"gemm16 tn {Bt}x[{K}x{M}x{N}]"):
        capi.check(lib.ssbev_gemm16_tn(capi.ptr(a16), capi.ptr(b16), capi.ptr(out), C.byref(d), capi.ptr(ws), ws.numel(),
                                       capi.stream()), "ssbev_gemm16_tn")
    return out


def _bmm16_tn(V, Z):
    if GEMM16_OWN and V.is_cuda:
        g = gemm16_tn(V, Z, tag=f"wino16 wgrad gemm {V.shape[0]}x[{V.shape[2]}x{V.shape[1]}x{Z.shape[2]}]")
        if g is not None:
            return g
    return torch.bmm(V.transpose(1, 2), Z, out_dtype=torch.float32)


def _wino_bgemm(V, w, Cout, Cin, mode):
    lib = capi.load()
    T, K = V.shape[1], V.shape[2]
    N = Cout if mode == 0 else Cin
    Wp = torch.empty(lib.ssbev_wino_dgemm_packed_elems(Cout, Cin), dtype=torch.float32, device=V.device)
    capi.check(lib.ssbev_wino_dgemm_pack(capi.ptr(w), capi.ptr(Wp), Cout, Cin, mode, capi.stream()), "ssbev_wino_dgemm_pack")
    M = torch.empty(64, T, N, dtype=torch.float32, device=V.device)
    capi.check(lib.ssbev_wino_bgemm(capi.ptr(V), capi.ptr(Wp), capi.ptr(M), T, K, N, capi.stream()), "ssbev_wino_bgemm")
    return M


def _wino_depth_fused(xcl, w, B, D, H, W, K, N, mode):
    lib = capi.load()
    Cout, Cin = (N, K) if mode == 0 else (K, N)
    R = B * D * (H // 2) * (W // 2)
    P = _wino_call("ssbev_wino2d_input_transform", xcl, capi.WinoDims(B, D, H, W, K), (16, R, K))
    Wp = torch.empty(lib.ssbev_wino_dgemm_packed_elems(Cout, Cin), dtype=torch.float32, device=xcl.device)
    capi.check(lib.ssbev_wino_dgemm_pack(capi.ptr(w), capi.ptr(Wp), Cout, Cin, mode, capi.stream()), "ssbev_wino_dgemm_pack")
    Mo = torch.empty(16, R, N, dtype=torch.float32, device=xcl.device)
    dims = capi.WinoDims(B, D, H, W, K)
    capi.check(lib.ssbev_wino_dgemm(capi.ptr(P), capi.ptr(Wp), capi.ptr(Mo), C.byref(dims), N, capi.stream()),
               "ssbev_wino_dgemm")
    del P
    return _wino_call("ssbev_wino2d_output_transform", Mo, capi.WinoDims(B, D, H, W, N), (B, D, H, W, N))


WINO_F43 = os.environ.get("SSBEV_WINO_F43", "1") != "0"
WINO_F43_2D = os.environ.get("SSBEV_WINO_F43_2D", "0") != "0"
WINO_F43_2D_DEPTHNET = os.environ.get("SSBEV_WINO_F43_2D_DEPTHNET", "0") != "0"
_F43_2D_SCOPE = 0


class wino_f43_2d_scope:

    def __enter__(self):
        global _F43_2D_SCOPE
        _F43_2D_SCOPE += 1 if WINO_F43_2D_DEPTHNET else 0
        return self

    def __exit__(self, *exc):
        global _F43_2D_SCOPE
        _F43_2D_SCOPE -= 1 if WINO_F43_2D_DEPTHNET else 0
        return False
WINO_F444 = os.environ.get("SSBEV_WINO_F444", "0") != "0"
WINO_F444_MIN_CIN = int(os.environ.get("SSBEV_WINO_F444_MIN_CIN", "0"))


WINO_DF = os.environ.get("SSBEV_WINO_DF", "1") != "0"
WINO_DF_MIN_ROWS = int(os.environ.get("SSBEV_WINO_DF_MIN_ROWS", "1024"))


def _wino_df_applicable(B, D, H, W, Cin, Cout):
    if not (WINO_DF and WINO_F43 and PRECISION == "fp32" and not (WINO_DEPTH_FUSED or WINO_OWN_GEMM or WINO_F444)):
        return False
    if B * D * (H // 4) * (W // 4) < WINO_DF_MIN_ROWS:
        return False
    lib = capi.load()
    return bool(lib.ssbev_wino43_df_supported(C.byref(capi.WinoDims(B, D, H, W, Cin)), Cout)) and \
        bool(lib.ssbev_wino43_df_supported(C.byref(capi.WinoDims(B, D, H, W, Cout)), Cin)) and Cout % 4 == 0


def _wino_df_gemm(xcl, w, B, D, H, W, K, N, mode, tag, fl, into=None):
    lib = capi.load()
    Cout, Cin = (N, K) if mode == 0 else (K, N)
    R = B * D * (H // 4) * (W // 4)
    with _span("wino_transform", 0.0, 4.0 * xcl.numel() * 3.25, tag + " in"):
        P = _wino_call("ssbev_wino43_2d_input_transform", xcl, capi.WinoDims(B, D, H, W, K), (36, R, K))
    Wp = torch.empty(lib.ssbev_wino43_df_packed_elems(Cout, Cin), dtype=torch.float32, device=xcl.device)
    capi.check(lib.ssbev_wino43_df_pack(capi.ptr(w), capi.ptr(Wp), Cout, Cin, mode, capi.stream()), "ssbev_wino43_df_pack")
    Mo = torch.empty(36, R, N, dtype=torch.float32, device=xcl.device)
    dims = capi.WinoDims(B, D, H, W, K)
    nby = 4.0 * (P.numel() + Mo.numel() + Wp.numel())
    with _span(f"conv_wino_fused:{lib.ssbev_wino43_df_instance(C.byref(dims), N)}" if KERNEL_TIMER is not None else "conv_wino_fused",
               fl, nby, tag, fl / 6.0):
        capi.check(lib.ssbev_wino43_df_gemm(capi.ptr(P), capi.ptr(Wp), capi.ptr(Mo), C.byref(dims), N, capi.stream()),
                   "ssbev_wino43_df_gemm")
    with _span("wino_transform", 0.0, 4.0 * B * D * H * W * N * (3.25 + (into is not None)), tag + " out"):
        if into is not None:
            odims = capi.WinoDims(B, D, H, W, N)
            capi.check(lib.ssbev_wino43_2d_output_transform_acc(capi.ptr(Mo), capi.ptr(into), C.byref(odims), capi.stream()),
                       "ssbev_wino43_2d_output_transform_acc")
            y = into
        else:
            y = _wino_call("ssbev_wino43_2d_output_transform", Mo, capi.WinoDims(B, D, H, W, N), (B, D, H, W, N))
    return y, P


class _WinoConvDF(torch.autograd.Function):

    @staticmethod
    def forward(ctx, x, weight, slot=None):
        ctx.slot = slot
        if ctx.needs_input_grad[1]:
            streams.note_use(weight)
        xcl = to_cl(_f32(x, "wino_conv"))
        B, D, H, W, Cin = xcl.shape
        Cout = weight.shape[0]
        fl = 2.0 * B * D * H * W * Cin * Cout * 27
        w = weight.detach().contiguous()
        y, P = _wino_df_gemm(xcl, w, B, D, H, W, Cin, Cout, 0, f"winoDF fwd {Cin}->{Cout} {D}x{H}x{W}", fl)
        ctx.save_for_backward(P if weight.requires_grad else None, weight)
        ctx.geom = (B, D, H, W, Cin, Cout, fl)
        return from_cl(y)

    @staticmethod
    def backward(ctx, gy):
        P, weight = ctx.saved_tensors
        B, D, H, W, Cin, Cout, fl = ctx.geom
        gcl = to_cl(gy)
        lib = capi.load()
        w = weight.detach().contiguous()
        gx = gw = None

        def weight_gradient():
            R = B * D * (H // 4) * (W // 4)
            with _span("wino_transform", 0.0, 4.0 * gcl.numel() * 3.25, "winoDF wgrad adjoint"):
                Z = _wino_call("ssbev_wino43_2d_output_adjoint", gcl, capi.WinoDims(B, D, H, W, Cout), (36, R, Cout))
            dims = capi.WinoDims(B, D, H, W, Cin)
            ws = _ws(lib.ssbev_wino43_df_wgrad_workspace(C.byref(dims), Cout), gy.device)
            gwt = torch.empty_like(w)
            nby = 4.0 * (P.numel() + Z.numel() + 144 * Cin * Cout)
            with _span("conv_wino_fused_wgrad", fl, nby, f"winoDF wgrad {Cin}->{Cout} {D}x{H}x{W}", fl / 6.0):
                capi.check(lib.ssbev_wino43_df_wgrad(capi.ptr(P), capi.ptr(Z), capi.ptr(gwt), C.byref(dims), Cout, capi.ptr(ws),
                                                     ws.numel(), capi.stream()), "ssbev_wino43_df_wgrad")
            return gwt

        gw_side = ctx.needs_input_grad[1] and streams.wgrad_on_side(weight)
        if gw_side:
            with streams.on_side(gy.device, gcl, P) as side:
                gw = weight_gradient()
                side.publish(gw)
        if ctx.needs_input_grad[0]:
            into = _slot_target(ctx.slot, torch.empty((B, D, H, W, Cin), device="meta"))
            gxcl, _ = _wino_df_gemm(gcl, w, B, D, H, W, Cout, Cin, 1, f"winoDF dgrad {Cin}->{Cout} {D}x{H}x{W}", fl, into=into)
            if ctx.slot is not None:
                ctx.slot.buf = gxcl
            gx = from_cl(gxcl)
        if ctx.needs_input_grad[1] and not gw_side:
            gw = weight_gradient()
        return gx, gw, None


class _WinoConv(torch.autograd.Function):

    @staticmethod
    def _plan(three_d, D, H, W, bf, cin=1 << 30):
        f43 = WINO_F43 and (three_d or WINO_F43_2D or _F43_2D_SCOPE > 0) and not bf and H % 4 == 0 and W % 4 == 0 and \
            not (three_d and (WINO_DEPTH_FUSED or WINO_OWN_GEMM))
        if f43 and three_d and WINO_F444 and D % 4 == 0 and cin >= WINO_F444_MIN_CIN:
            return 4, "ssbev_wino444_", 216, 4, 8.0
        if f43:
            pre = "ssbev_wino43_" if three_d else "ssbev_wino43_2d_"
            nf, th, reduction = (144, 4, 6.0) if three_d else (36, 4, 4.0)
        else:
            pre = "ssbev_wino_" if three_d else "ssbev_wino2d_"
            nf, th, reduction = (64, 2, 3.375) if three_d else (16, 2, 2.25)
        return (1 if f43 else 0), pre, nf, th, reduction

    @staticmethod
    def forward(ctx, x, weight, slot=None):
        ctx.slot = slot
        if ctx.needs_input_grad[1]:
            streams.note_use(weight)
        bf = PRECISION != "fp32"
        a16 = storage_bf16()
        xcl = to_cl(x if x.dtype == torch.bfloat16 else x.to(torch.bfloat16)) if a16 else to_cl(_f32(x, "wino_conv"))
        B, D, H, W, Cin = xcl.shape
        Cout, three_d = weight.shape[0], weight.shape[2] == 3
        f43, pre, nf, th, red = _WinoConv._plan(three_d, D, H, W, bf, Cin)
        T = B * (D // (4 if f43 == 4 else 2) if three_d else D) * (H // th) * (W // th)
        lib = capi.load()
        w = weight.detach().contiguous()
        fl = 2.0 * B * D * H * W * Cin * Cout * (27 if three_d else 9)
        fused = three_d and WINO_DEPTH_FUSED and not bf and not f43
        wt = lib.ssbev_wino43_weight_transform if f43 else lib.ssbev_wino_weight_transform
        wdim = 4 if f43 == 4 else (3 if three_d else 2)
        if not fused:
            U = torch.empty(nf, Cin, Cout, dtype=torch.float32, device=x.device)
            capi.check(wt(capi.ptr(w), capi.ptr(U), Cout, Cin, wdim, 0, capi.stream()), "ssbev_wino_weight_transform")
        tag = f"wino{ {0: '', 1: '43', 4: '444'}[f43]} fwd {Cin}->{Cout} {D}x{H}x{W}"
        nby = 4.0 * (B * D * H * W * (Cin + Cout) + (27 if three_d else 9) * Cin * Cout)
        with _span("conv_winograd", fl, nby, tag, fl / red):
            if fused:
                y = _wino_depth_fused(xcl, w, B, D, H, W, Cin, Cout, 0)
                V = None
            elif bf:
                sfx = "_bf16a" if a16 else "_bf16"
                V = _wino_call(pre + "input_transform" + sfx, xcl, capi.WinoDims(B, D, H, W, Cin), (nf, T, Cin), torch.bfloat16)
                M = _bmm16(V, U)
                y = _wino_call(pre + "output_transform" + sfx, M, capi.WinoDims(B, D, H, W, Cout), (B, D, H, W, Cout),
                               torch.bfloat16 if a16 else torch.float32)
            else:
                V = _wino_call(pre + "input_transform", xcl, capi.WinoDims(B, D, H, W, Cin), (nf, T, Cin))
                M = _wino_bgemm(V, w, Cout, Cin, 0) if (three_d and WINO_OWN_GEMM and not f43) else (gemm_nn(V, U, tag=tag + " gemm") if own_gemm_site("wino") else torch.bmm(V, U))
                y = _wino_call(pre + "output_transform", M, capi.WinoDims(B, D, H, W, Cout), (B, D, H, W, Cout))
        ctx.save_for_backward(xcl if fused else V, weight)
        ctx.geom = (B, D, H, W, Cin, Cout, T, three_d, fl, fused, bf, f43, pre, nf, red, a16)
        return from_cl(y)

    @staticmethod
    def backward(ctx, gy):
        V, weight = ctx.saved_tensors
        B, D, H, W, Cin, Cout, T, three_d, fl, fused, bf, f43, pre, nf, red, a16 = ctx.geom
        sfx, fdt = (("_bf16a" if a16 else "_bf16"), torch.bfloat16) if bf else ("", torch.float32)
        gcl = to_cl(gy)
        if a16 and gcl.dtype != torch.bfloat16:
            gcl = gcl.to(torch.bfloat16)
        adt = torch.bfloat16 if a16 else torch.float32
        lib = capi.load()
        w = weight.detach().contiguous()
        nd = 4 if f43 == 4 else (3 if three_d else 2)
        gx = gw = None
        vtag = {0: "", 1: "43", 4: "444"}[f43]
        nby = 4.0 * (B * D * H * W * (Cin + Cout) + (27 if three_d else 9) * Cin * Cout)
        if ctx.needs_input_grad[0] and fused:
            with _span("conv_winograd", fl, nby, f"wino dgrad {Cin}->{Cout} {D}x{H}x{W}", fl / red):
                gx = from_cl(_wino_depth_fused(gcl, w, B, D, H, W, Cout, Cin, 1))
        elif ctx.needs_input_grad[0]:
            Ut = torch.empty(nf, Cout, Cin, dtype=torch.float32, device=gy.device)
            wt = lib.ssbev_wino43_weight_transform if f43 else lib.ssbev_wino_weight_transform
            capi.check(wt(capi.ptr(w), capi.ptr(Ut), Cout, Cin, nd, 1, capi.stream()), "ssbev_wino_weight_transform")
            with _span("conv_winograd", fl, nby, f"wino{vtag} dgrad {Cin}->{Cout} {D}x{H}x{W}", fl / red):
                Vg = _wino_call(pre + "input_transform" + sfx, gcl, capi.WinoDims(B, D, H, W, Cout), (nf, T, Cout), fdt)
# ... 64 lines not shown
            capi.check(lib.ssbev_dcn_im2col(capi.ptr(xcl), capi.ptr(ocl), capi.ptr(cols), C.byref(d), capi.stream()),
                       "ssbev_dcn_im2col")
        ctx.save_for_backward(xcl, ocl)
        ctx.d = d
        return cols

    @staticmethod
    def backward(ctx, gcols):
        lib = capi.load()
        xcl, ocl = ctx.saved_tensors
        gx, goff = torch.empty_like(xcl), torch.empty_like(ocl)
        ws = _ws(lib.ssbev_dcn_col2im_workspace(C.byref(ctx.d)), xcl.device)
        with _span("dcn_sample", 0.0, 4.0 * (2 * xcl.numel() + 2 * ocl.numel() + gcols.numel()), "bwd   dcn_col2im"):
            capi.check(lib.ssbev_dcn_col2im(capi.ptr(xcl), capi.ptr(ocl), capi.ptr(gcols.contiguous()), capi.ptr(gx),
                                            capi.ptr(goff), C.byref(ctx.d), capi.ptr(ws), ws.numel(), capi.stream()),
                       "ssbev_dcn_col2im")
        return from_cl(gx), from_cl(goff), None, None, None, None


def deform_conv2d(x, offset, weight, groups=1, padding=1, dilation=1):
    Cout, Cg, k, _ = weight.shape
    B, _, H, W = x.shape
    cols = _DcnIm2col.apply(x, offset, int(groups), int(k), int(padding), int(dilation))
    Cog = Cout // groups
    Kc = k * k * Cg
    if (x.is_cuda and own_gemm_site("linear") and _gemm_supported(cols) and PRECISION == "fp32" and Cog % 4 == 0 and Kc % 4 == 0):
        w3 = weight.view(groups, Cog, Cg, k, k).permute(0, 1, 3, 4, 2).reshape(groups, Cog, Kc)
        y2 = _GroupedLinearCL.apply(cols, w3)
        return from_cl(y2.view(B, H, W, Cout))
    outs = []
    for g, cg in enumerate(cols.unbind(0)):
        colg = cg.view(B, H, W, Kc).permute(0, 3, 1, 2)
        wg = weight[g * Cog:(g + 1) * Cog].permute(0, 2, 3, 1).reshape(Cog, Kc, 1, 1)
        outs.append(conv2d(colg, wg, None, 1, 0, 1))
    return torch.cat(outs, dim=1) if groups > 1 else outs[0]


class _GroupedLinearCL(torch.autograd.Function):

    @staticmethod
    def forward(ctx, cols, w3):
        lib = capi.load()
        cols, w3 = cols.contiguous(), w3.contiguous()
        G, R, K = cols.shape
        N = w3.shape[1]
        y = torch.empty(R, G * N, dtype=torch.float32, device=cols.device)
        g = _gdims(R, N, K, G, K, K, G * N, R * K, N * K, N)
        ws = _ws(lib.ssbev_gemm_nt_workspace(C.byref(g)), cols.device)
        with _span("gemm_own", 2.0 * G * R * N * K, 4.0 * (cols.numel() + w3.numel() + y.numel()), f"linear fwd grouped {G}x[{K}->{N}] rows={R}"):
            capi.check(lib.ssbev_gemm_nt(capi.ptr(cols), capi.ptr(w3), None, capi.ptr(y), C.byref(g), capi.ptr(ws), ws.numel(),
                                         capi.stream()), "ssbev_gemm_nt")
        ctx.save_for_backward(cols, w3)
        return y

    @staticmethod
    def backward(ctx, gy):
        lib = capi.load()
        cols, w3 = ctx.saved_tensors
        G, R, K = cols.shape
        N = w3.shape[1]
        gy = gy.contiguous()
        gcols = gw = None
        fl = 2.0 * G * R * N * K
        if ctx.needs_input_grad[0]:
            gcols = torch.empty_like(cols)
            g = _gdims(R, K, N, G, G * N, K, K, N, N * K, R * K)
            ws = _ws(lib.ssbev_gemm_nn_workspace(C.byref(g)), gy.device)
            with _span("gemm_own", fl, 4.0 * (gy.numel() + w3.numel() + gcols.numel()), f"linear dgrad grouped {G}x[{K}->{N}] rows={R}"):
                capi.check(lib.ssbev_gemm_nn(capi.ptr(gy), capi.ptr(w3), None, capi.ptr(gcols), C.byref(g), capi.ptr(ws), ws.numel(),
                                             capi.stream()), "ssbev_gemm_nn")
        if ctx.needs_input_grad[1]:
            gw = torch.empty_like(w3)
            g = _gdims(R, K, N, G, G * N, K, K, N, R * K, N * K)
            ws = _ws(lib.ssbev_gemm_tn_workspace(C.byref(g)), gy.device)
            with _span("gemm_own", fl, 4.0 * (gy.numel() + cols.numel() + gw.numel()), f"linear wgrad grouped {G}x[{K}->{N}] rows={R}"):
                capi.check(lib.ssbev_gemm_tn(capi.ptr(gy), capi.ptr(cols), capi.ptr(gw), C.byref(g), capi.ptr(ws), ws.numel(),
                                             capi.stream()), "ssbev_gemm_tn")
        return gcols, gw




GN_RELU_MASK = os.environ.get("SSBEV_GN_RELU_MASK", "1") != "0"


def _norm_ext(device, running=None, n=0):
    e = capi.NormExt(None, None, 0.0, int(n))
    if running is not None:
        e.running_mean, e.running_var, e.momentum = running[0].data_ptr(), running[1].data_ptr(), float(running[2])
    return e


class _GroupNorm(torch.autograd.Function):

    @staticmethod
    def forward(ctx, x, weight, bias, residual, groups, eps, relu, as_batch, given_mean, given_rstd, pre_act=0, res_slot=None,
                running=None):
        lib = capi.load()
        ctx.res_slot = res_slot
        ctx.set_materialize_grads(False)
        xcl, io = _act(to_cl(x), "group_norm")
        Cch = xcl.shape[-1]
        B = 1 if as_batch else xcl.shape[0]
        S = xcl.numel() // (B * Cch)
        rcl = to_cl(residual if residual.dtype == xcl.dtype else residual.to(xcl.dtype)) if residual is not None else None
        given = given_mean is not None
        d = capi.NormDims(B, Cch, groups, S, float(eps), int(relu), int(given), int(pre_act), 0, 0, io)
        y = torch.empty_like(xcl)
        mean = given_mean.contiguous() if given else torch.empty(B * groups, dtype=torch.float32, device=x.device)
        rstd = given_rstd.contiguous() if given else torch.empty(B * groups, dtype=torch.float32, device=x.device)
        ws = _ws(lib.ssbev_groupnorm_workspace(C.byref(d)), x.device)
        w, b = weight.detach().contiguous(), bias.detach().contiguous()
        nb = float(xcl.element_size()) * xcl.numel() * (3 + (residual is not None) - 2 * given)
        use_mask = bool(relu) and GN_RELU_MASK and not given and any(ctx.needs_input_grad[:4])
        mask = torch.empty(lib.ssbev_groupnorm_mask_words(C.byref(d)), dtype=torch.int64, device=x.device) if use_mask else None
        ext = _norm_ext(x.device, running, B * S)
        with _span("groupnorm", 0.0, nb, f"fwd   N C={Cch} G={groups} S={S} res={int(residual is not None)}"):
            capi.check(lib.ssbev_groupnorm_fwd_ext(capi.ptr(xcl), capi.ptr(w), capi.ptr(b), capi.ptr(rcl), capi.ptr(y),
                                                   capi.ptr(mean), capi.ptr(rstd), capi.ptr(mask) if use_mask else None,
                                                   C.byref(d), C.byref(ext), capi.ptr(ws), ws.numel(), capi.stream()),
                       "ssbev_groupnorm_fwd_ext")
        ctx.save_for_backward(xcl, (mask if use_mask else y) if relu else None, w, mean, rstd)
        ctx.use_mask = use_mask
        ctx.meta = (B, S, Cch, groups, float(eps), int(relu), residual is not None, given, int(pre_act), io)
        ctx.mark_non_differentiable(mean, rstd)
        return from_cl(y), mean, rstd

    @staticmethod
    def backward(ctx, gy, _gm, _gr):
        lib = capi.load()
        xcl, y, w, mean, rstd = ctx.saved_tensors
        B, S, Cch, groups, eps, relu, has_res, given, pre_act, io = ctx.meta
        if given:
            raise capi.SsbevError("eval-mode (given statistics) normalisation has no HIP backward; use torch for it")
        gcl = to_cl(gy if gy.dtype == xcl.dtype else gy.to(xcl.dtype))
        d = capi.NormDims(B, Cch, groups, S, eps, relu, 0, pre_act, 0, 0, io)
        gx = torch.empty_like(xcl)
        gres = torch.empty_like(xcl) if has_res else None
        gg = torch.empty(Cch, dtype=torch.float32, device=gy.device)
        gb = torch.empty(Cch, dtype=torch.float32, device=gy.device)
        ws = _ws(lib.ssbev_groupnorm_workspace(C.byref(d)), gy.device)
        nb = float(xcl.element_size()) * xcl.numel() * (5 + (relu and not ctx.use_mask) + has_res)
        ext = _norm_ext(gy.device)
        with _span("groupnorm", 0.0, nb, f"bwd   N C={Cch} G={groups} S={S} res={int(has_res)}"):
            capi.check(lib.ssbev_groupnorm_bwd_ext(capi.ptr(gcl), capi.ptr(xcl), None if ctx.use_mask else capi.ptr(y),
                                                   capi.ptr(y) if ctx.use_mask else None, capi.ptr(w), capi.ptr(mean),
                                                   capi.ptr(rstd), capi.ptr(gx), capi.ptr(gres), capi.ptr(gg), capi.ptr(gb),
                                                   C.byref(d), C.byref(ext), capi.ptr(ws), ws.numel(), capi.stream()),
                       "ssbev_groupnorm_bwd_ext")
        if has_res and ctx.res_slot is not None and ctx.res_slot.buf is None:
            ctx.res_slot.buf = gres
        return from_cl(gx), gg, gb, (from_cl(gres) if has_res else None), None, None, None, None, None, None, None, None, None


NORM_CAT = os.environ.get("SSBEV_NORM_CAT", "1") != "0"


class _NormCat(torch.autograd.Function):

    @staticmethod
    def forward(ctx, parts, relu, running, *tensors):
        lib = capi.load()
        ctx.set_materialize_grads(False)
        n = len(parts)
        extra = tensors[3 * n] if len(tensors) > 3 * n else None
        xs = [to_cl(tensors[3 * i]) for i in range(n)]
        adt = xs[0].dtype if all(x.dtype == xs[0].dtype for x in xs) else torch.float32
        if adt == torch.bfloat16 and (any(x.shape[-1] % 8 for x in xs) or (extra is not None and extra.shape[1] % 8)):
            adt = torch.float32
        xs = [_act(x if x.dtype == adt else x.to(adt), "norm_cat")[0] for x in xs]
        io, esz = (1, 2) if adt == torch.bfloat16 else (0, 4)
        ws_ = [tensors[3 * i + 1].detach().contiguous() for i in range(n)]
        bs_ = [tensors[3 * i + 2].detach().contiguous() for i in range(n)]
        Cs = [x.shape[-1] for x in xs]
        Ctot = sum(Cs) + (extra.shape[1] if extra is not None else 0)
        out = torch.empty(xs[0].shape[:-1] + (Ctot,), dtype=adt, device=xs[0].device)
        if extra is not None:
            out[..., sum(Cs):].copy_(extra.detach().movedim(1, -1))
        saved, stats, metas = [], [], []
        c0 = 0
        for i, (groups, eps, as_batch) in enumerate(parts):
            x = xs[i]
            B = 1 if as_batch else x.shape[0]
            S = x.numel() // (B * Cs[i])
            d = capi.NormDims(B, Cs[i], groups, S, float(eps), int(relu), 0, 0, Ctot, 0, io)
            mean = torch.empty(B * groups, dtype=torch.float32, device=x.device)
            rstd = torch.empty(B * groups, dtype=torch.float32, device=x.device)
            ws = _ws(lib.ssbev_groupnorm_workspace(C.byref(d)), x.device)
            mask = torch.empty(lib.ssbev_groupnorm_mask_words(C.byref(d)), dtype=torch.int64, device=x.device) if relu else None
            run = running[i] if running is not None else None
            ext = _norm_ext(x.device, run, B * S)
            with _span("groupnorm", 0.0, 3.0 * esz * x.numel(), f"fwd   N C={Cs[i]} G={groups} S={S} cat@{c0}/{Ctot}"):
                capi.check(lib.ssbev_groupnorm_fwd_ext(capi.ptr(x), capi.ptr(ws_[i]), capi.ptr(bs_[i]), None,
                                                       C.c_void_p(out.data_ptr() + esz * c0), capi.ptr(mean), capi.ptr(rstd), capi.ptr(mask),
                                                       C.byref(d), C.byref(ext), capi.ptr(ws), ws.numel(), capi.stream()),
                           "ssbev_groupnorm_fwd_ext")
            saved += [x, mask, ws_[i], mean, rstd]
            stats += [mean, rstd]
            metas.append((B, S, Cs[i], groups, float(eps), c0))
            c0 += Cs[i]
        ctx.save_for_backward(*[t for t in saved if t is not None])
        ctx.has_mask = bool(relu)
        ctx.metas, ctx.relu, ctx.Ctot, ctx.io = metas, int(relu), Ctot, io
        ctx.extra_at = sum(Cs) if extra is not None else None
        ctx.mark_non_differentiable(*stats)
        return (from_cl(out), *stats)

    @staticmethod
    def backward(ctx, gy, *_):
        lib = capi.load()
        per = 5 if ctx.has_mask else 4
        sv = ctx.saved_tensors
        adt, esz = (torch.bfloat16, 2) if ctx.io else (torch.float32, 4)
        gcl = to_cl(gy if gy.dtype == adt else gy.to(adt))
        grads = []
        for i, (B, S, Cch, groups, eps, c0) in enumerate(ctx.metas):
            if ctx.has_mask:
                x, mask, w, mean, rstd = sv[per * i: per * i + 5]
            else:
                (x, w, mean, rstd), mask = sv[per * i: per * i + 4], None
            d = capi.NormDims(B, Cch, groups, S, eps, ctx.relu, 0, 0, 0, ctx.Ctot, ctx.io)
            gx = torch.empty_like(x)
            gg = torch.empty(Cch, dtype=torch.float32, device=gy.device)
            gb = torch.empty(Cch, dtype=torch.float32, device=gy.device)
            ws = _ws(lib.ssbev_groupnorm_workspace(C.byref(d)), gy.device)
            ext = _norm_ext(gy.device)
            with _span("groupnorm", 0.0, 5.0 * esz * x.numel(), f"bwd   N C={Cch} G={groups} S={S} cat@{c0}/{ctx.Ctot}"):
                capi.check(lib.ssbev_groupnorm_bwd_ext(C.c_void_p(gcl.data_ptr() + esz * c0), capi.ptr(x), None, capi.ptr(mask),
                                                       capi.ptr(w), capi.ptr(mean), capi.ptr(rstd), capi.ptr(gx), None, capi.ptr(gg),
                                                       capi.ptr(gb), C.byref(d), C.byref(ext), capi.ptr(ws), ws.numel(), capi.stream()),
                           "ssbev_groupnorm_bwd_ext")
            grads += [from_cl(gx), gg, gb]
        if ctx.extra_at is not None:
            grads.append(gcl[..., ctx.extra_at:].movedim(-1, 1))
        return (None, None, None, *grads)


def norm_cat(xs, norms, relu=True, extra=None, running=None):
    parts = tuple((int(g), float(e), bool(ab)) for (_, _, g, e, ab) in norms)
    flat = []
    for x, (w, b, _, _, _) in zip(xs, norms):
        flat += [x, w, b]
    if extra is not None:
        flat.append(extra)
    out = _NormCat.apply(parts, bool(relu), running, *flat)
    return out[0], [(out[1 + 2 * i], out[2 + 2 * i]) for i in range(len(xs))]


def norm_cat_supported(xs):
    return (NORM_CAT and GN_RELU_MASK and all(x.is_cuda and x.dtype in (torch.float32, torch.bfloat16) and x.shape[1] % 4 == 0 for x in xs)
            and all(x.shape[0] == xs[0].shape[0] and x.shape[2:] == xs[0].shape[2:] for x in xs))


def group_norm(x, groups, weight, bias, eps=1e-5, residual=None, relu=False, pre_act=None):
    if pre_act not in (None, "gelu"):
        raise ValueError(f"group_norm: unknown pre_act {pre_act!r}")
    return _GroupNorm.apply(x, weight, bias, residual, int(groups), eps, relu, False, None, None, 1 if pre_act else 0,
                            _slot_of(residual))[0]


def batch_norm_train(x, weight, bias, eps=1e-5, residual=None, relu=False, running=None):
    return _GroupNorm.apply(x, weight, bias, residual, x.shape[1], eps, relu, True, None, None, 0, _slot_of(residual), running)


def bn_update_running_(running_mean, running_var, mean, rstd, momentum, eps, n):
    lib = capi.load()
    capi.check(lib.ssbev_bn_update_running(capi.ptr(mean), capi.ptr(rstd), capi.ptr(running_mean), capi.ptr(running_var),
                                           running_mean.numel(), float(momentum), float(eps), int(n), capi.stream()),
               "ssbev_bn_update_running")


def batch_norm_eval(x, weight, bias, running_mean, running_var, eps=1e-5, residual=None, relu=False):
    rstd = torch.rsqrt(running_var + eps)
    return _GroupNorm.apply(x, weight, bias, residual, x.shape[1], eps, relu, True, running_mean, rstd)[0]


class _DualNorm(torch.autograd.Function):

    @staticmethod
    def forward(ctx, xa, wa, ba, xb, wb, bb, ga, gb, eps_a, eps_b, relu, a_batch, b_batch, run_a=None, run_b=None):
        lib = capi.load()
        ctx.set_materialize_grads(False)
        acl, io = _act(to_cl(xa), "dual_norm")
        bcl = to_cl(xb if xb.dtype == acl.dtype else xb.to(acl.dtype))
        if acl.shape != bcl.shape:
            raise capi.SsbevError(f"dual_norm: shapes differ, {tuple(acl.shape)} vs {tuple(bcl.shape)}")
        B, Cch = acl.shape[0], acl.shape[-1]
        S = acl.numel() // (B * Cch)
        d = capi.Norm2Dims(B, Cch, int(ga), int(gb), S, float(eps_a), float(eps_b), int(relu), int(a_batch), int(b_batch), io)
        dev = xa.device
        y = torch.empty_like(acl)
        mean_a = torch.empty((1 if a_batch else B) * ga, dtype=torch.float32, device=dev)
        rstd_a = torch.empty_like(mean_a)
        mean_b = torch.empty((1 if b_batch else B) * gb, dtype=torch.float32, device=dev)
        rstd_b = torch.empty_like(mean_b)
        nbytes = lib.ssbev_groupnorm2_workspace(C.byref(d))
        if nbytes == 0:
            raise capi.SsbevError("dual_norm: unsupported dims (C % 4, C <= 1024, C % G)")
        ws = _ws(nbytes, dev)
        nd = capi.NormDims(B, Cch, ga, S, float(eps_a), int(relu), 0, 0, 0, 0, io)
        mask = torch.empty(lib.ssbev_groupnorm_mask_words(C.byref(nd)), dtype=torch.int64, device=dev) if relu else None
        wa_, ba_, wb_, bb_ = (t.detach().contiguous() for t in (wa, ba, wb, bb))
        ext = capi.Norm2Ext(None, None, 0.0, None, None, 0.0)
        if run_a is not None and a_batch:
            ext.running_mean_a, ext.running_var_a, ext.momentum_a = run_a[0].data_ptr(), run_a[1].data_ptr(), float(run_a[2])
        if run_b is not None and b_batch:
            ext.running_mean_b, ext.running_var_b, ext.momentum_b = run_b[0].data_ptr(), run_b[1].data_ptr(), float(run_b[2])
        with _span("groupnorm", 0.0, float(acl.element_size()) * acl.numel() * 5, f"fwd   N2 C={Cch} Ga={ga} Gb={gb} S={S}"):
            capi.check(lib.ssbev_groupnorm2_fwd_ext(capi.ptr(acl), capi.ptr(wa_), capi.ptr(ba_), capi.ptr(mean_a), capi.ptr(rstd_a),
                                                    capi.ptr(bcl), capi.ptr(wb_), capi.ptr(bb_), capi.ptr(mean_b), capi.ptr(rstd_b),
                                                    capi.ptr(y), capi.ptr(mask), C.byref(d), C.byref(ext), capi.ptr(ws), ws.numel(),
                                                    capi.stream()),
                       "ssbev_groupnorm2_fwd_ext")
        ctx.save_for_backward(acl, bcl, mask, wa_, wb_, mean_a, rstd_a, mean_b, rstd_b)
        ctx.meta = (B, Cch, int(ga), int(gb), S, float(eps_a), float(eps_b), int(relu), int(a_batch), int(b_batch), io)
        ctx.mark_non_differentiable(mean_a, rstd_a, mean_b, rstd_b)
        return from_cl(y), mean_a, rstd_a, mean_b, rstd_b

    @staticmethod
    def backward(ctx, gy, *_unused):
        lib = capi.load()
        acl, bcl, mask, wa_, wb_, mean_a, rstd_a, mean_b, rstd_b = ctx.saved_tensors
        d = capi.Norm2Dims(*ctx.meta)
        Cch, dev = ctx.meta[1], gy.device
        gcl = to_cl(gy if gy.dtype == acl.dtype else gy.to(acl.dtype))
        gxa, gxb = torch.empty_like(acl), torch.empty_like(bcl)
        gga, gba, ggb, gbb = (torch.empty(Cch, dtype=torch.float32, device=dev) for _ in range(4))
        ws = _ws(lib.ssbev_groupnorm2_workspace(C.byref(d)), dev)
        with _span("groupnorm", 0.0, float(acl.element_size()) * acl.numel() * 8, f"bwd   N2 C={Cch} Ga={ctx.meta[2]} Gb={ctx.meta[3]} S={ctx.meta[4]}"):
            ext = capi.Norm2Ext(None, None, 0.0, None, None, 0.0)
            capi.check(lib.ssbev_groupnorm2_bwd_ext(capi.ptr(gcl), capi.ptr(mask), capi.ptr(acl), capi.ptr(wa_), capi.ptr(mean_a),
                                                    capi.ptr(rstd_a), capi.ptr(bcl), capi.ptr(wb_), capi.ptr(mean_b), capi.ptr(rstd_b),
                                                    capi.ptr(gxa), capi.ptr(gxb), capi.ptr(gga), capi.ptr(gba), capi.ptr(ggb),
                                                    capi.ptr(gbb), C.byref(d), C.byref(ext), capi.ptr(ws), ws.numel(), capi.stream()),
                       "ssbev_groupnorm2_bwd_ext")
        return from_cl(gxa), gga, gba, from_cl(gxb), ggb, gbb, None, None, None, None, None, None, None, None, None


DUAL_NORM = os.environ.get("SSBEV_DUAL_NORM", "1") != "0"


# ... 408 lines not shown
```

stereoscene_amd/layers.py:

```python
import math

import torch
import torch.nn as nn

from . import functional as F


def _ntuple(v, n):
    return (v,) * n if isinstance(v, int) else tuple(v)


class _ConvBase(nn.Module):
    ND = 3
    TRANSPOSED = False

    def __init__(self, in_channels, out_channels, kernel_size, stride=1, padding=0, dilation=1, groups=1,
                 bias=True, output_padding=0):
        super().__init__()
        if groups != 1:
            raise NotImplementedError("grouped convolution is only provided by DeformConv2dPack")
        n = self.ND
        self.in_channels, self.out_channels = in_channels, out_channels
        self.kernel_size = _ntuple(kernel_size, n)
        self.stride, self.padding = _ntuple(stride, n), _ntuple(padding, n)
        self.dilation, self.output_padding = _ntuple(dilation, n), _ntuple(output_padding, n)
        shape = ((in_channels, out_channels) if self.TRANSPOSED else (out_channels, in_channels)) + self.kernel_size
        self.weight = nn.Parameter(torch.empty(shape))
        self.bias = nn.Parameter(torch.empty(out_channels)) if bias else None
        self.reset_parameters()

    def reset_parameters(self):
        nn.init.kaiming_uniform_(self.weight, a=math.sqrt(5))
        if self.bias is not None:
            fan_in = self.weight[0].numel() if not self.TRANSPOSED else self.weight.shape[0] * self.weight[0, 0].numel()
            bound = 1 / math.sqrt(max(fan_in, 1))
            nn.init.uniform_(self.bias, -bound, bound)

    def extra_repr(self):
        return (f"{self.in_channels}, {self.out_channels}, kernel_size={self.kernel_size}, stride={self.stride}, "
                f"padding={self.padding}, hip=mfma_f32_32x32x2")


class Conv3d(_ConvBase):
    def forward(self, x, relu=False):
        return F.conv3d(x, self.weight, self.bias, self.stride, self.padding, self.dilation, relu=relu)


class ConvTranspose3d(_ConvBase):
    TRANSPOSED = True

    def __init__(self, in_channels, out_channels, kernel_size, stride=1, padding=0, output_padding=0, bias=True):
        super().__init__(in_channels, out_channels, kernel_size, stride, padding, 1, 1, bias, output_padding)

    def forward(self, x):
        return F.conv_transpose3d(x, self.weight, self.bias, self.stride, self.padding, self.output_padding)


class Conv2d(_ConvBase):
    ND = 2

    def forward(self, x):
        return F.conv2d(x, self.weight, self.bias, self.stride, self.padding, self.dilation)


class DeformConv2dPack(nn.Module):

    def __init__(self, in_channels, out_channels, kernel_size=3, stride=1, padding=1, dilation=1, groups=1,
                 deform_groups=1, im2col_step=128, bias=False):
        super().__init__()
        assert not bias and deform_groups == 1 and stride == 1
        self.groups, self.k, self.padding, self.dilation = groups, kernel_size, padding, dilation
        self.weight = nn.Parameter(torch.empty(out_channels, in_channels // groups, kernel_size, kernel_size))
        self.conv_offset = Conv2d(in_channels, 2 * kernel_size * kernel_size, kernel_size, 1, padding, dilation)
        n = in_channels * kernel_size * kernel_size
        nn.init.uniform_(self.weight, -1 / math.sqrt(n), 1 / math.sqrt(n))
        nn.init.zeros_(self.conv_offset.weight)
        nn.init.zeros_(self.conv_offset.bias)

    def forward(self, x):
        return F.deform_conv2d(x, self.conv_offset(x), self.weight, self.groups, self.padding, self.dilation)

    def _forward_reference(self, x, off):
        B, C, H, W = x.shape
        k, K = self.k, self.k * self.k
        dev = x.device
        base_h = (torch.arange(H, device=dev, dtype=x.dtype) - self.padding)[:, None]
        base_w = (torch.arange(W, device=dev, dtype=x.dtype) - self.padding)[None, :]
        ki = torch.arange(K, device=dev)
        off = off.reshape(B, K, 2, H, W)
        hh = base_h + (ki // k * self.dilation).view(1, K, 1, 1).to(x.dtype) + off[:, :, 0]
        ww = base_w + (ki % k * self.dilation).view(1, K, 1, 1).to(x.dtype) + off[:, :, 1]
        inside = (hh > -1) & (ww > -1) & (hh < H) & (ww < W)
        h0, w0 = torch.floor(hh), torch.floor(ww)
        lh, lw = hh - h0, ww - w0
        flat = x.reshape(B, C, H * W)
        cols = 0
        for dh, dw, wt in ((0, 0, (1 - lh) * (1 - lw)), (0, 1, (1 - lh) * lw), (1, 0, lh * (1 - lw)), (1, 1, lh * lw)):
            hi, wi = (h0 + dh).long(), (w0 + dw).long()
            ok = inside & (hi >= 0) & (hi < H) & (wi >= 0) & (wi < W)
            lin = (hi.clamp(0, H - 1) * W + wi.clamp(0, W - 1)).view(B, 1, K * H * W).expand(B, C, K * H * W)
            g = torch.gather(flat, 2, lin).view(B, C, K, H * W)
            cols = cols + g * (wt * ok).view(B, 1, K, H * W)
        G = self.groups
        cols = cols.view(B, G, (C // G) * K, H * W)
        wmat = self.weight.view(G, self.weight.shape[0] // G, -1)
        out = torch.einsum("gok,bgkn->bgon", wmat, cols)
        return out.reshape(B, self.weight.shape[0], H, W)


class GroupNorm(nn.GroupNorm):
    fused_relu = False

    def forward(self, x, residual=None, relu=None):
        relu = self.fused_relu if relu is None else relu
        if x.dim() < 3 or self.num_channels % 4 != 0:
            y = nn.functional.group_norm(x, self.num_groups, self.weight, self.bias, self.eps)
            y = y if residual is None else y + residual
            return torch.relu(y) if relu else y
        return F.group_norm(x, self.num_groups, self.weight, self.bias, self.eps, residual, relu)


class _HipBatchNorm:
    fused_relu = False

    def _running(self):
        if not self.track_running_stats:
            return None
        with torch.no_grad():
            m = self.momentum if self.momentum is not None else 1.0 / float(self.num_batches_tracked + 1)
            self.num_batches_tracked += 1
        return (self.running_mean, self.running_var, m)

    def forward(self, x, residual=None, relu=None):
        relu = self.fused_relu if relu is None else relu
        if self.training:
            y, mean, rstd = F.batch_norm_train(x, self.weight, self.bias, self.eps, residual, relu, running=self._running())
            return y
        if torch.is_grad_enabled() and (x.requires_grad or self.weight.requires_grad):
            shape = (1, -1) + (1,) * (x.dim() - 2)
            scale = self.weight * torch.rsqrt(self.running_var + self.eps)
            y = x * scale.view(shape) + (self.bias - self.running_mean * scale).view(shape)
            y = y if residual is None else y + residual
            return torch.relu(y) if relu else y
        return F.batch_norm_eval(x, self.weight, self.bias, self.running_mean, self.running_var, self.eps, residual,
                                 relu)


class BatchNorm3d(_HipBatchNorm, nn.BatchNorm3d):
    pass


class BatchNorm2d(_HipBatchNorm, nn.BatchNorm2d):
    pass


def norm_pair(norm_a, xa, norm_b, xb, relu=True):
    def fusable(n):
        return isinstance(n, GroupNorm) or (isinstance(n, _HipBatchNorm) and n.training)
    if not (F.DUAL_NORM and fusable(norm_a) and fusable(norm_b) and F.dual_norm_supported(xa, xb)):
        return norm_a(xa, residual=norm_b(xb), relu=relu)

    def side(n):
        if isinstance(n, GroupNorm):
            return n.num_groups, False
        return n.num_features, True
    (ga, a_batch), (gb, b_batch) = side(norm_a), side(norm_b)
    run = [n._running() if isinstance(n, _HipBatchNorm) else None for n in (norm_a, norm_b)]
    y, sa, sb = F.dual_norm(xa, norm_a.weight, norm_a.bias, ga, norm_a.eps, xb, norm_b.weight, norm_b.bias, gb, norm_b.eps,
                            relu=relu, a_batch=a_batch, b_batch=b_batch, running_a=run[0], running_b=run[1])
    return y


def norm_cat(norms, xs, relu=True, extra=None):
    def fusable(n):
        return isinstance(n, GroupNorm) or (isinstance(n, _HipBatchNorm) and n.training)
    if not (all(fusable(n) for n in norms) and F.norm_cat_supported(list(xs))
            and (extra is None or (extra.is_cuda and extra.shape[1] % 4 == 0))):
        ys = [n(x, relu=relu) for n, x in zip(norms, xs)]
        return torch.cat(ys + ([extra] if extra is not None else []), dim=1)
    spec = [(n.weight, n.bias, n.num_groups, n.eps, False) if isinstance(n, GroupNorm)
            else (n.weight, n.bias, n.num_features, n.eps, True) for n in norms]
    run = tuple(n._running() if isinstance(n, _HipBatchNorm) else None for n in norms)
    y, stats = F.norm_cat(list(xs), spec, relu=relu, extra=extra, running=run)
    return y


def _last_leaf(m):
    while isinstance(m, nn.Sequential) and len(m) > 0:
        m = m[len(m) - 1]
    return m


def fuse_relu_(module):
    for seq in [m for m in module.modules() if isinstance(m, nn.Sequential)]:
        for i in range(1, len(seq)):
            prev = _last_leaf(seq[i - 1])
            if isinstance(seq[i], nn.ReLU) and isinstance(prev, (GroupNorm, BatchNorm3d, BatchNorm2d)):
                prev.fused_relu = True
                seq[i] = nn.Identity()
    return module


def build_norm_layer(cfg, num_features, postfix=""):
    cfg = dict(cfg)
    t = cfg.pop("type")
    requires_grad = cfg.pop("requires_grad", True)
    if t == "GN":
        name, layer = "gn", GroupNorm(cfg["num_groups"], num_features, eps=cfg.get("eps", 1e-5))
    elif t in ("BN", "BN2d"):
        name, layer = "bn", BatchNorm2d(num_features)
    elif t == "BN3d":
        name, layer = "bn", BatchNorm3d(num_features)
    else:
        raise KeyError(f"unsupported norm type {t}")
    for p in layer.parameters():
        p.requires_grad = requires_grad
    return name + str(postfix), layer


def build_conv_layer(cfg, *args, **kwargs):
    cfg = dict(cfg) if cfg else dict(type="Conv2d")
    t = cfg.pop("type")
    kwargs = {**cfg, **kwargs}
    table = {"Conv2d": Conv2d, "Conv": Conv2d, "Conv3d": Conv3d, "DCN": DeformConv2dPack}
    if t not in table:
        raise KeyError(f"unsupported conv type {t}")
    return table[t](*args, **kwargs)


def build_upsample_layer(cfg, *args, **kwargs):
    cfg = dict(cfg)
    t = cfg.pop("type")
    kwargs = {**cfg, **kwargs}
    if t != "deconv3d":
        raise KeyError(f"unsupported upsample type {t}")
    return ConvTranspose3d(*args, **kwargs)
```

stereoscene_amd/plugin/voxel_encoder.py:

```python
import numpy as np
import torch
import torch.nn as nn

from .. import functional as F
from ..layers import Conv3d, GroupNorm, build_conv_layer, build_norm_layer, build_upsample_layer, fuse_relu_, norm_pair
from ..registry import BACKBONES, HEADS, NECKS
from . import losses as L


class BasicBlock3d(nn.Module):
    expansion = 1

    def __init__(self, in_planes, planes, stride=1, downsample=None, norm_cfg=None):
        super().__init__()
        self.conv1 = Conv3d(in_planes, planes, 3, stride, 1, bias=False)
        self.bn1 = build_norm_layer(norm_cfg, planes)[1]
        self.conv2 = Conv3d(planes, planes, 3, 1, 1, bias=False)
        self.bn2 = build_norm_layer(norm_cfg, planes)[1]
        self.downsample = downsample
        self.stride = stride

    def forward(self, x):
        xa, xb = F.fork(x)
        out = self.bn1(self.conv1(xa), relu=True)
        if self.downsample is None:
            return self.bn2(self.conv2(out), residual=xb, relu=True)
        return norm_pair(self.bn2, self.conv2(out), self.downsample[1], self.downsample[0](xb), relu=True)


@BACKBONES.register_module()
class CustomResNet3D(nn.Module):
    def __init__(self, depth, block_inplanes=(64, 128, 256, 512), block_strides=(1, 2, 2, 2), out_indices=(0, 1, 2, 3),
                 num_stage=4, n_input_channels=3, shortcut_type="B", norm_cfg=dict(type="BN3d", requires_grad=True),
                 crp3d=False, crp_level=2, widen_factor=1.0):
        super().__init__()
        if depth not in (10, 18, 34) or crp3d or shortcut_type != "B":
            raise NotImplementedError("only the BasicBlock / shortcut-B / no-CRP variants used by the config are built")
        nblocks = {10: [1, 1, 1, 1], 18: [2, 2, 2, 2], 34: [3, 4, 6, 3]}[depth]
        planes = [int(c * widen_factor) for c in block_inplanes]
        self.in_planes = planes[0]
        self.out_indices, self.num_stage, self.crp3d = out_indices, num_stage, False
        self.input_proj = nn.Sequential(Conv3d(n_input_channels, self.in_planes, 1, 1, 0, bias=False),
                                        build_norm_layer(norm_cfg, self.in_planes)[1], nn.ReLU(inplace=True))
        self.layers = nn.ModuleList()
        for i, c in enumerate(planes[:num_stage]):
            self.layers.append(self._make_layer(c, nblocks[i], block_strides[i], norm_cfg))
        fuse_relu_(self)
        for m in self.modules():
            if isinstance(m, Conv3d):
                nn.init.kaiming_normal_(m.weight, mode="fan_out", nonlinearity="relu")

    def _make_layer(self, planes, blocks, stride, norm_cfg):
        down = None
        if stride != 1 or self.in_planes != planes:
            down = nn.Sequential(Conv3d(self.in_planes, planes, 1, stride, 0, bias=False),
                                 build_norm_layer(norm_cfg, planes)[1])
        layers = [BasicBlock3d(self.in_planes, planes, stride, down, norm_cfg)]
        self.in_planes = planes
        layers += [BasicBlock3d(planes, planes, norm_cfg=norm_cfg) for _ in range(1, blocks)]
        return nn.Sequential(*layers)

    def forward(self, x):
        x = self.input_proj(x)
        res = []
        for i, layer in enumerate(self.layers):
            x = layer(x)
            if i in self.out_indices:
                if i + 1 < len(self.layers):
                    x, out = F.fork(x)
                    res.append(out)
                else:
                    res.append(x)
        return res


@NECKS.register_module()
class SECONDFPN3D(nn.Module):
    def __init__(self, in_channels=(128, 128, 256), out_channels=(256, 256, 256), upsample_strides=(1, 2, 4),
                 norm_cfg=dict(type="GN", num_groups=32, requires_grad=True),
                 upsample_cfg=dict(type="deconv3d", bias=False), conv_cfg=dict(type="Conv3d", bias=False),
                 use_conv_for_no_stride=False, use_output_upsample=False, with_cp=False, init_cfg=None):
        super().__init__()
        assert len(out_channels) == len(upsample_strides) == len(in_channels) and not use_output_upsample
        self.in_channels, self.out_channels = list(in_channels), list(out_channels)
        blocks = []
        for cin, cout, s in zip(in_channels, out_channels, upsample_strides):
            if s >= 1 and not (s == 1 and use_conv_for_no_stride):
                up = build_upsample_layer(upsample_cfg, in_channels=cin, out_channels=cout, kernel_size=s, stride=s)
            else:
                k = int(np.round(1 / s))
                up = build_conv_layer(conv_cfg, in_channels=cin, out_channels=cout, kernel_size=k, stride=k)
            blocks.append(nn.Sequential(up, build_norm_layer(norm_cfg, cout)[1], nn.ReLU(inplace=True)))
        self.deblocks = nn.ModuleList(blocks)
        fuse_relu_(self)

    def forward(self, x):
        assert len(x) == len(self.in_channels)
        norms = [blk[1] for blk in self.deblocks]
        if (len(x) > 1 and all(isinstance(n, GroupNorm) and n.fused_relu for n in norms)
                and all(isinstance(blk[2], nn.Identity) for blk in self.deblocks)):
            raw = [blk[0](f) for blk, f in zip(self.deblocks, x)]
            if F.norm_cat_supported(raw):
                return [F.norm_cat(raw, [(n.weight, n.bias, n.num_groups, n.eps, False) for n in norms], relu=True)[0]]
# ... 60 lines not shown
```

Measured before the change: 30.63 million voxels/s.

## Compute GroupNorm partial statistics in Winograd output-transform epilogue

```diff
diff --git a/include/ssbev.h b/include/ssbev.h
--- a/include/ssbev.h
+++ b/include/ssbev.h
@@ -145,6 +145,10 @@
                             const float* mean, const float* rstd, float* gx, float* gresidual, float* ggamma, float* gbeta,
                             const ssbev_norm_dims* d, const ssbev_norm_ext* ext, void* ws, size_t ws_bytes,
                             ssbev_stream_t stream);
+
+int ssbev_groupnorm_fwd_records(const float* x, const float* gamma, const float* beta, const float* residual, float* y,
+                                float* mean, float* rstd, uint64_t* relu_mask, const float* records, int64_t nrec,
+                                const ssbev_norm_dims* d, void* ws, size_t ws_bytes, ssbev_stream_t stream);
 
 typedef struct { int B, C, Ga, Gb; int64_t S; float eps_a, eps_b; int relu; int a_batch, b_batch; int io_dtype;  } ssbev_norm2_dims;
 size_t ssbev_groupnorm2_workspace(const ssbev_norm2_dims* d);
@@ -276,6 +280,9 @@
 int ssbev_wino43_2d_input_transform(const float* x, float* V, const ssbev_wino_dims* d, ssbev_stream_t stream);
 int ssbev_wino43_2d_output_transform(const float* M, float* y, const ssbev_wino_dims* d, ssbev_stream_t stream);
 int ssbev_wino43_2d_output_transform_acc(const float* M, float* y, const ssbev_wino_dims* d, ssbev_stream_t stream);
+int64_t ssbev_wino43_2d_output_stats_chunks(const ssbev_wino_dims* d, int G);
+int ssbev_wino43_2d_output_transform_stats(const float* M, float* y, float* records, int G, const ssbev_wino_dims* d,
+                                           ssbev_stream_t stream);
 int ssbev_wino2d_output_transform_acc(const float* M, float* y, const ssbev_wino_dims* d, ssbev_stream_t stream);
 int ssbev_wino43_2d_output_adjoint(const float* gy, float* Z, const ssbev_wino_dims* d, ssbev_stream_t stream);
 int ssbev_wino43_input_transform_bf16(const float* x, uint16_t* V, const ssbev_wino_dims* d, ssbev_stream_t stream);
diff --git a/stereoscene_amd/capi.py b/stereoscene_amd/capi.py
--- a/stereoscene_amd/capi.py
+++ b/stereoscene_amd/capi.py
@@ -143,6 +143,7 @@
     "ssbev_groupnorm_bwd_mask": (C.c_int, [_P] * 10 + [C.POINTER(NormDims), _P, C.c_size_t, _P]),
     "ssbev_groupnorm_fwd_ext": (C.c_int, [_P] * 8 + [C.POINTER(NormDims), C.POINTER(NormExt), _P, C.c_size_t, _P]),
     "ssbev_groupnorm_bwd_ext": (C.c_int, [_P] * 11 + [C.POINTER(NormDims), C.POINTER(NormExt), _P, C.c_size_t, _P]),
+    "ssbev_groupnorm_fwd_records": (C.c_int, [_P] * 9 + [C.c_int64, C.POINTER(NormDims), _P, C.c_size_t, _P]),
     "ssbev_groupnorm2_fwd_ext": (C.c_int, [_P] * 12 + [C.POINTER(Norm2Dims), C.POINTER(Norm2Ext), _P, C.c_size_t, _P]),
     "ssbev_groupnorm2_bwd_ext": (C.c_int, [_P] * 16 + [C.POINTER(Norm2Dims), C.POINTER(Norm2Ext), _P, C.c_size_t, _P]),
     "ssbev_groupnorm2_workspace": (C.c_size_t, [C.POINTER(Norm2Dims)]),
@@ -208,6 +209,8 @@
     "ssbev_wino43_2d_input_transform_bf16": (C.c_int, [_P, _P, C.POINTER(WinoDims), _P]),
     "ssbev_wino43_2d_output_transform": (C.c_int, [_P, _P, C.POINTER(WinoDims), _P]),
     "ssbev_wino43_2d_output_transform_acc": (C.c_int, [_P, _P, C.POINTER(WinoDims), _P]),
+    "ssbev_wino43_2d_output_stats_chunks": (C.c_int64, [C.POINTER(WinoDims), C.c_int]),
+    "ssbev_wino43_2d_output_transform_stats": (C.c_int, [_P, _P, _P, C.c_int, C.POINTER(WinoDims), _P]),
     "ssbev_wino2d_output_transform_acc": (C.c_int, [_P, _P, C.POINTER(WinoDims), _P]),
     "ssbev_wino43_2d_output_transform_bf16": (C.c_int, [_P, _P, C.POINTER(WinoDims), _P]),
     "ssbev_wino43_2d_output_adjoint": (C.c_int, [_P, _P, C.POINTER(WinoDims), _P]),
diff --git a/stereoscene_amd/csrc/groupnorm.hip b/stereoscene_amd/csrc/groupnorm.hip
--- a/stereoscene_amd/csrc/groupnorm.hip
+++ b/stereoscene_amd/csrc/groupnorm.hip
@@ -243,6 +243,40 @@
     double var = sq / n - m * m;
     if (var < 0.0) var = 0.0;
     mean[blockIdx.x] = (float)m;
+    rstd[blockIdx.x] = (float)(1.0 / sqrt(var + (double)g.eps));
+  }
+}
+
+__global__ void __launch_bounds__(FT)
+gn_finalize_rec_kernel(const float4* __restrict__ rec, long nrec, float* __restrict__ mean, float* __restrict__ rstd,
+                       GnGeom g) {
+  __shared__ double s0[FT / 64], s1[FT / 64];
+  const float4* rb = rec + (size_t)blockIdx.x * nrec;
+  const double pg = rb[0].z;
+  double a[4] = {0, 0, 0, 0}, q[4] = {0, 0, 0, 0};
+  constexpr int kFinBatch = 8;
+  for (long i0 = threadIdx.x; i0 < nrec; i0 += (long)kFinBatch * FT) {
+    float4 r[kFinBatch];
+#pragma unroll
+    for (int k = 0; k < kFinBatch; ++k) {
+      const long i = i0 + (long)k * FT;
+      r[k] = i < nrec ? rb[i] : make_float4(0.f, 0.f, 0.f, 0.f);
+    }
+#pragma unroll
+    for (int k = 0; k < kFinBatch; ++k) {
+      const double dp = (double)r[k].z - pg, n = r[k].w;
+      a[k & 3] += (double)r[k].x + n * dp;
+      q[k & 3] += (double)r[k].y + 2.0 * dp * (double)r[k].x + n * dp * dp;
+    }
+  }
+  double sa = (a[0] + a[1]) + (a[2] + a[3]), sq = (q[0] + q[1]) + (q[2] + q[3]);
+  block_sum2(sa, sq, s0, s1);
+  if (threadIdx.x == 0) {
+    const double n = (double)g.S * (g.C / g.G);
+    const double md = sa / n;
+    double var = sq / n - md * md;
+    if (var < 0.0) var = 0.0;
+    mean[blockIdx.x] = (float)(pg + md);
     rstd[blockIdx.x] = (float)(1.0 / sqrt(var + (double)g.eps));
   }
 }
@@ -951,6 +985,22 @@
                              size_t ws_bytes, ssbev_stream_t stream) {
   if (d && d->relu && !relu_mask) return SSBEV_EINVAL;
   return groupnorm_fwd_impl(x, gamma, beta, residual, y, mean, rstd, reinterpret_cast<unsigned long long*>(relu_mask), d, ws,
+                            ws_bytes, stream);
+}
+
+int ssbev_groupnorm_fwd_records(const float* x, const float* gamma, const float* beta, const float* residual, float* y,
+                                float* mean, float* rstd, uint64_t* relu_mask, const float* records, int64_t nrec,
+                                const ssbev_norm_dims* d, void* ws, size_t ws_bytes, ssbev_stream_t stream) {
+  if (!gn_ok(d) || d->io_dtype != 0 || d->pre_act != 0 || d->stats_given || !records || nrec <= 0) return SSBEV_EINVAL;
+  if (d->relu && !relu_mask) return SSBEV_EINVAL;
+  if (!x || !gamma || !beta || !y || !mean || !rstd) return SSBEV_EINVAL;
+  if (reinterpret_cast<uintptr_t>(records) % 16 != 0) return SSBEV_EINVAL;
+  const GnGeom g = make_geom(d);
+  hipLaunchKernelGGL(gn_finalize_rec_kernel, dim3(g.B * g.G), dim3(FT), 0, as_stream(stream),
+                     reinterpret_cast<const float4*>(records), (long)nrec, mean, rstd, g);
+  ssbev_norm_dims dg = *d;
+  dg.stats_given = 1;
+  return groupnorm_fwd_impl(x, gamma, beta, residual, y, mean, rstd, reinterpret_cast<unsigned long long*>(relu_mask), &dg, ws,
                             ws_bytes, stream);
 }
 
diff --git a/stereoscene_amd/csrc/winograd.hip b/stereoscene_amd/csrc/winograd.hip
--- a/stereoscene_amd/csrc/winograd.hip
+++ b/stereoscene_amd/csrc/winograd.hip
@@ -573,6 +573,69 @@
         y[(((long)b * g.H + 4 * th + e) * g.W + 4 * tw + f) * g.C + c] = r2[e * 4 + f];
       }
     }
+}
+
+__global__ void __launch_bounds__(1024)
+wino43_output_stats_kernel(const float* __restrict__ M, float* __restrict__ y, float* __restrict__ rec, WinoGeom g, int G,
+                           int tpi, int nchunk) {
+  extern __shared__ __align__(16) double dl[];
+  const int nthr = blockDim.x, tid = threadIdx.x, r = tid / g.C, c = tid % g.C, cpg = g.C / G;
+  double* da = dl;
+  double* dq = dl + g.C;
+  float* fa = reinterpret_cast<float*>(dl + 2 * g.C);
+  float* fq = fa + nthr;
+  float* piv = fq + nthr;
+  const int chunk = blockIdx.x, b = blockIdx.y;
+  const long Ts = (long)g.D * (g.H / 4) * (g.W / 4);
+  const long tl = (long)chunk * tpi + r;
+  const bool act = r < tpi && tl < Ts;
+  float o[16];
+#pragma unroll
+  for (int k = 0; k < 16; ++k) o[k] = 0.0f;
+  if (act) {
+    const long tile = (long)b * Ts + tl, T = (long)g.B * Ts;
+    const int tw = (int)(tile % (g.W / 4));
+    const long t1 = tile / (g.W / 4);
+    const int th = (int)(t1 % (g.H / 4));
+    const long pl = t1 / (g.H / 4);
+    float m[36];
+#pragma unroll
+    for (int xi = 0; xi < 36; ++xi) m[xi] = M[((long)xi * T + tile) * g.C + c];
+    float r1[24];
+#pragma unroll
+    for (int p = 0; p < 6; ++p) at6(m + p * 6, 1, r1 + p * 4, 1);
+#pragma unroll
+    for (int f = 0; f < 4; ++f) at6(r1 + f, 4, o + f, 4);
+#pragma unroll
+    for (int e = 0; e < 4; ++e)
+#pragma unroll
+      for (int f = 0; f < 4; ++f) y[((pl * g.H + 4 * th + e) * g.W + 4 * tw + f) * g.C + c] = o[e * 4 + f];
+    if (r == 0 && c % cpg == 0) piv[c / cpg] = o[0];
+  }
+  __syncthreads();
+  float a = 0.0f, q = 0.0f;
+  if (act) {
+    const float p = piv[c / cpg];
+#pragma unroll
+    for (int k = 0; k < 16; ++k) { const float dv = o[k] - p; a += dv; q += dv * dv; }
+  }
+  fa[tid] = a;
+  fq[tid] = q;
+  __syncthreads();
+  if (tid < g.C) {
+    double sa = 0.0, sq = 0.0;
+    for (int rr = 0; rr < tpi; ++rr) { sa += fa[rr * g.C + tid]; sq += fq[rr * g.C + tid]; }
+    da[tid] = sa;
+    dq[tid] = sq;
+  }
+  __syncthreads();
+  if (tid < G) {
+    double sa = 0.0, sq = 0.0;
+    for (int k = 0; k < cpg; ++k) { sa += da[tid * cpg + k]; sq += dq[tid * cpg + k]; }
+    const long ntile = min((long)tpi, Ts - (long)chunk * tpi);
+    *reinterpret_cast<float4*>(rec + (((long)b * G + tid) * nchunk + chunk) * 4) =
+        make_float4((float)sa, (float)sq, piv[tid], (float)(16L * cpg * ntile));
+  }
 }
 
 template <int DA, typename TF>
@@ -1053,6 +1116,28 @@
 SSBEV_WINO43_ENTRY(ssbev_wino444_output_transform, wino43_output_kernel, 4, float, float, float)
 SSBEV_WINO43_ENTRY(ssbev_wino444_output_adjoint, wino43_output_adjoint_kernel, 4, float, float, float)
 
+static int wino43_stats_tpi(int C) { return C >= 256 ? 1 : 256 / C; }
+
+int64_t ssbev_wino43_2d_output_stats_chunks(const ssbev_wino_dims* d, int G) {
+  if (!wino43_ok(d, 0) || G <= 0 || d->C % G != 0 || d->C > 1024) return 0;
+  const long Ts = (long)d->D * (d->H / 4) * (d->W / 4);
+  const int tpi = wino43_stats_tpi(d->C);
+  return (Ts + tpi - 1) / tpi;
+}
+
+int ssbev_wino43_2d_output_transform_stats(const float* src, float* dst, float* records, int G, const ssbev_wino_dims* d,
+                                           ssbev_stream_t stream) {
+  const int64_t nchunk = ssbev_wino43_2d_output_stats_chunks(d, G);
+  if (nchunk <= 0 || nchunk > 0x7fffffff || !src || !dst || !records) return SSBEV_EINVAL;
+  const int tpi = wino43_stats_tpi(d->C);
+  const int nthr = (tpi * d->C + 63) / 64 * 64;
+  const size_t lds = 2 * (size_t)d->C * sizeof(double) + (2 * (size_t)nthr + G) * sizeof(float);
+  const WinoGeom g{d->B, d->D, d->H, d->W, d->C};
+  hipLaunchKernelGGL(wino43_output_stats_kernel, dim3((unsigned)nchunk, d->B), dim3(nthr), lds, as_stream(stream), src, dst,
+                     records, g, G, tpi, (int)nchunk);
+  return ssbev_launch_status();
+}
+
 int ssbev_wino43_2d_output_transform_acc(const float* src, float* dst, const ssbev_wino_dims* d, ssbev_stream_t stream) {
   if (!wino43_ok(d, 0) || !src || !dst) return SSBEV_EINVAL;
   const long total = (long)d->B * d->D * (d->H / 4) * (d->W / 4) * d->C;
diff --git a/stereoscene_amd/functional.py b/stereoscene_amd/functional.py
--- a/stereoscene_amd/functional.py
+++ b/stereoscene_amd/functional.py
@@ -754,7 +754,7 @@
 WINO_BF16S = os.environ.get("SSBEV_WINO_BF16S", "1") != "0"
 
 
-def conv3d(x, weight, bias=None, stride=1, padding=0, dilation=1, relu=False):
+def conv3d(x, weight, bias=None, stride=1, padding=0, dilation=1, relu=False, norm_groups=None):
     st, pd, dl = _triple(stride, 3), _triple(padding, 3), _triple(dilation, 3)
     if storage_bf16() and x.is_cuda and TILE_HINT in (0, 7, 9):
         if WIDE16 and _wide16_applicable(x, weight, st, pd, dl):
@@ -780,7 +780,10 @@
         B, Cin, D, H, W = x.shape
         if tuple(weight.shape[2:]) == (3, 3, 3) and H % 4 == 0 and W % 4 == 0 and \
                 _wino_df_applicable(B, D, H, W, Cin, weight.shape[0]):
-            y = _WinoConvDF.apply(x, weight, _slot_of(x))
+            stats = _epilogue_records(B, D, H, W, weight.shape[0], norm_groups, x.device) if bias is None else None
+            y = _WinoConvDF.apply(x, weight, _slot_of(x), stats)
+            if stats is not None:
+                _attach_records(y, stats)
         else:
             y = _WinoConv.apply(x, weight, _slot_of(x))
         return y if bias is None else y + bias.view(1, -1, 1, 1, 1)
@@ -1226,7 +1229,7 @@
         bool(lib.ssbev_wino43_df_supported(C.byref(capi.WinoDims(B, D, H, W, Cout)), Cin)) and Cout % 4 == 0
 
 
-def _wino_df_gemm(xcl, w, B, D, H, W, K, N, mode, tag, fl, into=None):
+def _wino_df_gemm(xcl, w, B, D, H, W, K, N, mode, tag, fl, into=None, stats=None):
     lib = capi.load()
     Cout, Cin = (N, K) if mode == 0 else (K, N)
     R = B * D * (H // 4) * (W // 4)
@@ -1247,6 +1250,11 @@
             capi.check(lib.ssbev_wino43_2d_output_transform_acc(capi.ptr(Mo), capi.ptr(into), C.byref(odims), capi.stream()),
                        "ssbev_wino43_2d_output_transform_acc")
             y = into
+        elif stats is not None:
+            y = torch.empty(B, D, H, W, N, dtype=torch.float32, device=xcl.device)
+            capi.check(lib.ssbev_wino43_2d_output_transform_stats(capi.ptr(Mo), capi.ptr(y), capi.ptr(stats[0]), int(stats[1]),
+                                                                  C.byref(capi.WinoDims(B, D, H, W, N)), capi.stream()),
+                       "ssbev_wino43_2d_output_transform_stats")
         else:
             y = _wino_call("ssbev_wino43_2d_output_transform", Mo, capi.WinoDims(B, D, H, W, N), (B, D, H, W, N))
     return y, P
@@ -1255,7 +1263,7 @@
 class _WinoConvDF(torch.autograd.Function):
 
     @staticmethod
-    def forward(ctx, x, weight, slot=None):
+    def forward(ctx, x, weight, slot=None, stats=None):
         ctx.slot = slot
         if ctx.needs_input_grad[1]:
             streams.note_use(weight)
@@ -1264,7 +1272,7 @@
         Cout = weight.shape[0]
         fl = 2.0 * B * D * H * W * Cin * Cout * 27
         w = weight.detach().contiguous()
-        y, P = _wino_df_gemm(xcl, w, B, D, H, W, Cin, Cout, 0, f"winoDF fwd {Cin}->{Cout} {D}x{H}x{W}", fl)
+        y, P = _wino_df_gemm(xcl, w, B, D, H, W, Cin, Cout, 0, f"winoDF fwd {Cin}->{Cout} {D}x{H}x{W}", fl, stats=stats)
         ctx.save_for_backward(P if weight.requires_grad else None, weight)
         ctx.geom = (B, D, H, W, Cin, Cout, fl)
         return from_cl(y)
@@ -1304,7 +1312,7 @@
             gx = from_cl(gxcl)
         if ctx.needs_input_grad[1] and not gw_side:
             gw = weight_gradient()
-        return gx, gw, None
+        return gx, gw, None, None
 
 
 class _WinoConv(torch.autograd.Function):
@@ -1535,6 +1543,30 @@
 
 
 GN_RELU_MASK = os.environ.get("SSBEV_GN_RELU_MASK", "1") != "0"
+GN_EPILOGUE_STATS = os.environ.get("SSBEV_GN_EPILOGUE_STATS", "1") != "0"
+
+
+def _epilogue_records(B, D, H, W, N, groups, device):
+    if not GN_EPILOGUE_STATS or not groups or N % int(groups) != 0:
+        return None
+    nrec = int(capi.load().ssbev_wino43_2d_output_stats_chunks(C.byref(capi.WinoDims(B, D, H, W, N)), int(groups)))
+    if nrec <= 0:
+        return None
+    return (torch.empty(B * int(groups) * nrec * 4, dtype=torch.float32, device=device), int(groups), nrec)
+
+
+def _attach_records(y, stats):
+    y._ssbev_gn_records = (stats, y._version)
+
+
+def _take_records(x, groups):
+    r = getattr(x, "_ssbev_gn_records", None)
+    if r is None:
+        return None
+    (rec, g, nrec), ver = r
+    if g != groups or ver != x._version or not GN_EPILOGUE_STATS:
+        return None
+    return rec, nrec
 
 
 def _norm_ext(device, running=None, n=0):
@@ -1548,7 +1580,7 @@
 
     @staticmethod
     def forward(ctx, x, weight, bias, residual, groups, eps, relu, as_batch, given_mean, given_rstd, pre_act=0, res_slot=None,
-                running=None):
+                running=None, records=None):
         lib = capi.load()
         ctx.res_slot = res_slot
         ctx.set_materialize_grads(False)
@@ -1568,11 +1600,21 @@
         use_mask = bool(relu) and GN_RELU_MASK and not given and any(ctx.needs_input_grad[:4])
         mask = torch.empty(lib.ssbev_groupnorm_mask_words(C.byref(d)), dtype=torch.int64, device=x.device) if use_mask else None
         ext = _norm_ext(x.device, running, B * S)
+        from_records = records is not None and not given and not as_batch and not pre_act and io == 0
+        if from_records:
+            nb -= float(xcl.element_size()) * xcl.numel()
         with _span("groupnorm", 0.0, nb, f"fwd   N C={Cch} G={groups} S={S} res={int(residual is not None)}"):
-            capi.check(lib.ssbev_groupnorm_fwd_ext(capi.ptr(xcl), capi.ptr(w), capi.ptr(b), capi.ptr(rcl), capi.ptr(y),
-                                                   capi.ptr(mean), capi.ptr(rstd), capi.ptr(mask) if use_mask else None,
-                                                   C.byref(d), C.byref(ext), capi.ptr(ws), ws.numel(), capi.stream()),
-                       "ssbev_groupnorm_fwd_ext")
+            if from_records:
+                capi.check(lib.ssbev_groupnorm_fwd_records(capi.ptr(xcl), capi.ptr(w), capi.ptr(b), capi.ptr(rcl), capi.ptr(y),
+                                                           capi.ptr(mean), capi.ptr(rstd), capi.ptr(mask) if use_mask else None,
+                                                           capi.ptr(records[0]), int(records[1]), C.byref(d), capi.ptr(ws),
+                                                           ws.numel(), capi.stream()),
+                           "ssbev_groupnorm_fwd_records")
+            else:
+                capi.check(lib.ssbev_groupnorm_fwd_ext(capi.ptr(xcl), capi.ptr(w), capi.ptr(b), capi.ptr(rcl), capi.ptr(y),
+                                                       capi.ptr(mean), capi.ptr(rstd), capi.ptr(mask) if use_mask else None,
+                                                       C.byref(d), C.byref(ext), capi.ptr(ws), ws.numel(), capi.stream()),
+                           "ssbev_groupnorm_fwd_ext")
         ctx.save_for_backward(xcl, (mask if use_mask else y) if relu else None, w, mean, rstd)
         ctx.use_mask = use_mask
         ctx.meta = (B, S, Cch, groups, float(eps), int(relu), residual is not None, given, int(pre_act), io)
@@ -1603,7 +1645,7 @@
                        "ssbev_groupnorm_bwd_ext")
         if has_res and ctx.res_slot is not None and ctx.res_slot.buf is None:
             ctx.res_slot.buf = gres
-        return from_cl(gx), gg, gb, (from_cl(gres) if has_res else None), None, None, None, None, None, None, None, None, None
+        return from_cl(gx), gg, gb, (from_cl(gres) if has_res else None), None, None, None, None, None, None, None, None, None, None
 
 
 NORM_CAT = os.environ.get("SSBEV_NORM_CAT", "1") != "0"
@@ -1709,7 +1751,7 @@
     if pre_act not in (None, "gelu"):
         raise ValueError(f"group_norm: unknown pre_act {pre_act!r}")
     return _GroupNorm.apply(x, weight, bias, residual, int(groups), eps, relu, False, None, None, 1 if pre_act else 0,
-                            _slot_of(residual))[0]
+                            _slot_of(residual), None, None if pre_act else _take_records(x, int(groups)))[0]
 
 
 def batch_norm_train(x, weight, bias, eps=1e-5, residual=None, relu=False, running=None):
diff --git a/stereoscene_amd/layers.py b/stereoscene_amd/layers.py
--- a/stereoscene_amd/layers.py
+++ b/stereoscene_amd/layers.py
@@ -42,8 +42,11 @@
 
 
 class Conv3d(_ConvBase):
+    norm_groups = None
+
     def forward(self, x, relu=False):
-        return F.conv3d(x, self.weight, self.bias, self.stride, self.padding, self.dilation, relu=relu)
+        return F.conv3d(x, self.weight, self.bias, self.stride, self.padding, self.dilation, relu=relu,
+                        norm_groups=None if relu else self.norm_groups)
 
 
 class ConvTranspose3d(_ConvBase):
@@ -191,8 +194,16 @@
     return m
 
 
+def link_norm_stats_(conv, norm):
+    if isinstance(conv, Conv3d) and isinstance(norm, GroupNorm):
+        conv.norm_groups = norm.num_groups
+    return conv
+
+
 def fuse_relu_(module):
     for seq in [m for m in module.modules() if isinstance(m, nn.Sequential)]:
+        for i in range(1, len(seq)):
+            link_norm_stats_(seq[i - 1], seq[i])
         for i in range(1, len(seq)):
             prev = _last_leaf(seq[i - 1])
             if isinstance(seq[i], nn.ReLU) and isinstance(prev, (GroupNorm, BatchNorm3d, BatchNorm2d)):
diff --git a/stereoscene_amd/plugin/voxel_encoder.py b/stereoscene_amd/plugin/voxel_encoder.py
--- a/stereoscene_amd/plugin/voxel_encoder.py
+++ b/stereoscene_amd/plugin/voxel_encoder.py
@@ -3,7 +3,8 @@
 import torch.nn as nn
 
 from .. import functional as F
-from ..layers import Conv3d, GroupNorm, build_conv_layer, build_norm_layer, build_upsample_layer, fuse_relu_, norm_pair
+from ..layers import (Conv3d, GroupNorm, build_conv_layer, build_norm_layer, build_upsample_layer, fuse_relu_, link_norm_stats_,
+                      norm_pair)
 from ..registry import BACKBONES, HEADS, NECKS
 from . import losses as L
 
@@ -19,6 +20,9 @@
         self.bn2 = build_norm_layer(norm_cfg, planes)[1]
         self.downsample = downsample
         self.stride = stride
+        link_norm_stats_(self.conv1, self.bn1)
+        if downsample is None:
+            link_norm_stats_(self.conv2, self.bn2)
 
     def forward(self, x):
         xa, xb = F.fork(x)
```

After: 30.72 million voxels/s (median of 6 runs). No clear change (+0.3%).
